# tangtang888/video-edge-ai-proxy

Measured on AMD Instinct MI355X. Metric: decoded FPS (whole node) + p50 VideoLatestImage latency, 256×1080p RTSP, higher is better.
Workload: dtype uint8 (BGR24 frames; bf16-capable consumer path)

## Files before the change

csrc/bindings.cpp:

```cpp
#include <malloc.h>

#include <pybind11/numpy.h>
#include <pybind11/pybind11.h>
#include <pybind11/stl.h>

#include "vep/hostprof.h"
#include "vep/avc.h"
#include "vep/avc_cavlc.h"
#include "vep/avc_recon.h"
#include "vep/bench_driver.h"
#include "vep/cabac.h"
#include "vep/codec.h"
#include "vep/gpu.h"
#include "vep/h264.h"
#include "vep/hevc_ctu.h"
#include "vep/hevc_dec.h"
#include "vep/hevc_kern.h"
#include "vep/jpeg.h"
#include "vep/scale.h"
#include "bind_ext.h"
#include "vep/runtime.h"
#include "vep/synth.h"

namespace py = pybind11;
// ... 113 lines not shown
  py::array_t<uint32_t> counts({py::ssize_t(r.rows), py::ssize_t(r.cols)});
  std::memcpy(counts.mutable_data(), r.counts.data(), r.counts.size() * sizeof(uint32_t));
  d["counts"] = counts;
  return d;
}

struct CpuDecoder {
  StreamParser parser;
  MbUpdate upd;
  HostSurface surf;
  PictureInfo last;
  avc::Decoder avc;
  std::vector<HostSurface> slots;
  bool general = false;
  int target = 0;
  int coded = 0;
  bool fields_out = false;
  HostSurface woven;
  mutable HostSurface weave_tmp;
  const HostSurface& out() const { return general ? (fields_out ? woven : slots[size_t(target)]) : surf; }
  const HostSurface& frame_of(const avc::OutFrame& f) const {
    if (!f.fields) return slots[size_t(f.slot)];
    avc::weave_fields(slots[2 * size_t(f.slot)], slots[2 * size_t(f.slot) + 1], weave_tmp);
    return weave_tmp;
  }
  py::object decode(const AccessUnit& au) {
    bool no_output = false;
    {
      py::gil_scoped_release nogil;
      bool done = false;
      if (!general) {
        try {
          upd.clear_payload();
          last = parser.parse(au, upd);
          if (surf.coded_w != last.coded_width || surf.coded_h != last.coded_height)
            surf.alloc(last.coded_width, last.coded_height);
          cpu_apply_update(upd, surf);
          coded = upd.nslots;
          done = true;
        } catch (const UnsupportedStream&) {
          if (au.codec != Codec::kH264) throw;
          general = true;
        }
      }
      std::vector<avc::OutFrame> outs;
      size_t nal = 0;
      while (!done) {
        avc::PicturePtr pic = avc.parse(au, 0, &nal);
        done = nal >= au.nals.size();
        if (slots.size() < size_t(pic->dpb_slots)) slots.resize(size_t(pic->dpb_slots));
        for (auto& h : slots)
          if (h.coded_w != pic->wmbs * 16 || h.coded_h != pic->hmbs * 16 || h.bd != pic->bd || h.cf != pic->cf)
            h.alloc(pic->wmbs * 16, pic->hmbs * 16, pic->bd, pic->cf);
        avc::cpu_reconstruct(*pic, slots);
        coded = pic->info.coded_mbs;
        pictures.push_back(pic->info);
        for (const avc::MbRec& m : pic->mbs) {
          ++kinds[m.kind];
          if (m.flags & avc::kMbT8x8) ++t8x8;
          if (m.flags & avc::kMbWp) ++weighted;
          if (m.kind <= avc::kInter) {
            bool bi = false, l1only = false;
            for (int k = 0; k < 4; ++k) {
              bi |= m.ref[k] != 0xFF && m.ref1[k] != 0xFF;
              l1only |= m.ref[k] == 0xFF && m.ref1[k] != 0xFF;
            }
            bipred += bi;
            list1_only += l1only;
          }
        }
        outs.insert(outs.end(), pic->outputs.begin(), pic->outputs.end());
        if (!done) continue;
        pending_outputs = outs;
        no_output = outs.empty();
        if (!no_output) {
          last = outs.back().info;
          target = outs.back().slot;
          fields_out = outs.back().fields;
          if (fields_out) woven = frame_of(outs.back());
          last_poc = outs.back().poc;
          last_pts = outs.back().au.pts;
        }
      }
    }
    if (no_output) return py::none();
    py::array_t<uint8_t> o({last.height, last.width, 3});
    cpu_nv12_to_bgr(out(), last.crop_left, last.crop_top, last.width, last.height, o.mutable_data());
    return o;
  }
  py::list frames_of(const std::vector<avc::OutFrame>& fs) const {
    py::list l;
    for (const auto& f : fs) {
      const HostSurface& s = frame_of(f);
      l.append(py::make_tuple(f.au.pts, surface_planes(s)));
    }
    return l;
  }
  py::list flush() {
    py::list out_list;
    for (const auto& f : avc.flush_output()) {
      py::array_t<uint8_t> o({f.info.height, f.info.width, 3});
      cpu_nv12_to_bgr(frame_of(f), f.info.crop_left, f.info.crop_top, f.info.width, f.info.height,
                      o.mutable_data());
      out_list.append(o);
    }
    return out_list;
// ... 668 lines not shown
        for (int i = 0; i < 16; ++i) want[256 + 16 * k + i] = res.blk[16 + k][i] = coded ? val(dens) : 0;
        if (coded) res.chroma |= u8(1u << k);
      }
      avc::Picture pic;
      pic.wmbs = pic.hmbs = 1;
      pic.mbs.resize(1);
      avc::MbRec rec{};
      rec.kind = res.t8 ? avc::kI8x8 : avc::kI16x16;
      rec.flags = res.t8 ? u8(avc::kMbT8x8) : u8(0);
      avc::MbState s;
      avc::store_mb(pic, 0, rec, s, &res, nullptr);
      i16 got[avc::kDenseCoefs];
      avc::expand_coefs(pic.coefs.data(), pic.mbs[0], got);
      bad_avc += std::memcmp(got, want, sizeof got) != 0 ||
                 pic.coefs.size() != size_t(avc::coef_words(pic.mbs[0])) + avc::coef_values(pic.coefs.data(), pic.mbs[0]);
      for (int log2 = 2; log2 <= 5; ++log2) {
        const int nn = 1 << (2 * log2);
        std::vector<i16> dense(size_t(nn), 0), val_list, out(size_t(nn + nn / 16)), back(static_cast<size_t>(nn));
        std::vector<u16> pos;
        for (int k = 0; k < nn; ++k)
          if ((dense[size_t(k)] = val(dens))) pos.push_back(u16(k));
        for (size_t i = pos.size(); i > 1; --i) std::swap(pos[i - 1], pos[size_t(rnd() % i)]);
        for (u16 k : pos) val_list.push_back(dense[k]);
        const int n = hevc::hk_sparse_store(log2, pos.data(), val_list.data(), int(pos.size()), out.data());
        hevc::hk_sparse_expand(out.data(), log2, back.data());
        bad_hevc += back != dense || n != hevc::hk_sparse_words(log2) + int(pos.size());
      }
    }
    return std::make_pair(bad_avc, bad_hevc);
  });
  m.def("avc_parse_seconds", [](const std::vector<std::shared_ptr<AccessUnit>>& aus, int reps) {
    py::gil_scoped_release r;
    double best = 1e30;
    for (int k = 0; k < std::max(1, reps); ++k) {
      avc::Decoder dec;
      const i64 t0 = mono_us();
      for (const auto& au : aus) {
        size_t nal = 0;
        do dec.parse(*au, 0, &nal);
        while (nal < au->nals.size());
      }
      best = std::min(best, double(mono_us() - t0) * 1e-6);
    }
    return best;
  }, py::arg("aus"), py::arg("reps") = 3);
  m.def("avc_record_stats", [](const std::vector<std::shared_ptr<AccessUnit>>& aus) {
    py::gil_scoped_release r;
    avc::Decoder dec;
    u64 mbs = 0, coefs = 0, nz = 0, mvs = 0, pics = 0;
    for (const auto& au : aus) {
      auto p = dec.parse(*au);
      if (!p) continue;
      ++pics;
      mbs += p->mbs.size();
      coefs += p->coefs.size();
      mvs += p->mvs.size();
      for (const avc::MbRec& m : p->mbs)
        if (m.kind != avc::kIPcm) nz += avc::coef_values(p->coefs.data(), m);
    }
    py::gil_scoped_acquire g;
    py::dict d;
    d["pictures"] = pics;
    d["mbs"] = mbs;
    d["coefs"] = coefs;
    d["nonzero"] = nz;
    d["mvs"] = mvs;
    return d;
  });
  m.def("hevc_record_stats", [](const std::vector<std::shared_ptr<AccessUnit>>& aus) {
    py::gil_scoped_release r;
    hevc::Decoder dec;
    dec.set_gpu_mode(true);
    u64 pics = 0, tus = 0, coefs = 0, nz = 0, pus = 0;
    for (const auto& au : aus) {
      dec.decode(*au);
      for (const auto& p : dec.take_gpu_pictures()) {
        ++pics;
        tus += p->tus.size();
        pus += p->pus.size();
        coefs += p->coefs.size();
        for (i16 c : p->coefs) nz += c != 0;
      }
    }
    py::gil_scoped_acquire g;
    py::dict d;
    d["pictures"] = pics;
    d["tus"] = tus;
    d["coefs"] = coefs;
    d["nonzero"] = nz;
    d["pus"] = pus;
    return d;
  });
  m.def("avc_intra8x8_tap_check", [](u64 seed, int trials) {
    u64 st = seed * 0x9E3779B97F4A7C15ull + 7;
    auto rnd = [&]() {
      st ^= st << 13;
      st ^= st >> 7;
      st ^= st << 17;
      return int(st & 255);
    };
    int bad = 0;
    for (int t = 0; t < trials; ++t) {
      int s[25];
      for (int k = 0; k < 25; ++k) s[k] = (t & 3) == 0 ? (rnd() & 1) * 255 : rnd();
      auto T = [&](int i) { return s[1 + i]; };
      auto L = [&](int j) { return j < 0 ? s[0] : s[17 + j]; };
// ... 1064 lines not shown
          return tiles;
        },
        py::arg("pics"), py::arg("stream"));
  m.def("letterbox",
        [](uintptr_t y, uintptr_t uv, int pitch, int src_w, int src_h, int crop_left, int crop_top,
           int size, uintptr_t out_hwc, uintptr_t out_chw, int chw_dtype, std::vector<float> mean,
           std::vector<float> stdv, int pad, uintptr_t stream, int format) {
          gpu::LetterboxDesc d{};
          d.y = reinterpret_cast<const u8*>(y);
          d.uv = reinterpret_cast<const u8*>(uv);
          d.pitch = pitch;
          d.src_w = src_w;
          d.src_h = src_h;
          d.crop_left = crop_left;
          d.crop_top = crop_top;
          d.out_hwc = reinterpret_cast<u8*>(out_hwc);
          d.out_chw = reinterpret_cast<void*>(out_chw);
          gpu::LetterboxParams p{};
          p.format = format;
          p.size = size;
          p.chw_dtype = chw_dtype;
          for (int k = 0; k < 3; ++k) {
            p.mean[k] = mean.size() == 3 ? mean[size_t(k)] : 0.f;
            p.inv_std[k] = 1.f / (stdv.size() == 3 ? stdv[size_t(k)] : 1.f);
          }
          p.pad_value = u8(pad);
          gpu::check_letterbox(d, p);
          gpu::fill_letterbox_geometry(d, size, format == gpu::kLbNV12);
          gpu::launch_letterbox_one(d, p, reinterpret_cast<hipStream_t>(stream));
        },
        py::arg("y"), py::arg("uv"), py::arg("pitch"), py::arg("src_w"), py::arg("src_h"),
        py::arg("crop_left"), py::arg("crop_top"), py::arg("size"), py::arg("out_hwc"),
        py::arg("out_chw"), py::arg("chw_dtype"), py::arg("mean"), py::arg("std"), py::arg("pad"),
        py::arg("stream"), py::arg("format") = 0);
  m.def("nv12_to_chw",
        [](uintptr_t in, uintptr_t out, int n, int size, int chw_dtype, std::vector<float> mean,
           std::vector<float> stdv, uintptr_t stream) {
          float m3[3], is3[3];
          for (int k = 0; k < 3; ++k) {
            m3[k] = mean.size() == 3 ? mean[size_t(k)] : 0.f;
            is3[k] = 1.f / (stdv.size() == 3 ? stdv[size_t(k)] : 1.f);
          }
          gpu::launch_nv12_to_chw(reinterpret_cast<const u8*>(in), reinterpret_cast<void*>(out), n,
                                  size, chw_dtype, m3, is3, reinterpret_cast<hipStream_t>(stream));
        });
  m.def("letterbox_geometry", [](int src_w, int src_h, int size, bool even) {
    gpu::LetterboxDesc d{};
    d.src_w = src_w;
    d.src_h = src_h;
    gpu::fill_letterbox_geometry(d, size, even);
    return py::make_tuple(d.nw, d.nh, d.pad_x, d.pad_y);
  }, py::arg("src_w"), py::arg("src_h"), py::arg("size"), py::arg("even") = false);

  bind_net(m);
  bind_mux(m);
  bind_hevc(m);
  bind_bus(m);
  bind_rpc(m);
}
```

csrc/vep/avc.cpp:

```cpp
#include "avc.h"

#include <immintrin.h>

#include <algorithm>
#include <array>

#include "avc_cavlc.h"
#include "avc_internal.h"
#include "fanout.h"

namespace vep::avc {

using h264::Pps;
using h264::Sps;


void MbNeighbours::reset(int wmbs, int hmbs, bool ring) {
  w_ = wmbs;
  h_ = hmbs;
  cur_ = -1;
  run_slice_ = ~0u;
  run_start_ = 0;
  announced_ = 0;
  const size_t n = size_t(wmbs) * hmbs;
  if (++epoch_ == 0) {
    epoch_ = 1;
    stamp_.clear();
  }
  size_t ns = n;
  mask_ = ~size_t(0);
  if (ring) {
    size_t r = 1;
    while (r < 2 * (size_t(wmbs) + 2)) r <<= 1;
    if (r < n) {
      ns = r;
      mask_ = r - 1;
    }
  }
  if (st_.size() != ns) st_.assign(ns, MbState{});
  if (tag_.size() != ns) tag_.assign(ns, ~0u);
  if (stamp_.size() != n) stamp_.assign(n, 0u);
}

static int coded_count(const MbState& s, int blk) {
  if (s.kind == kSkip) return 0;
  if (s.kind == kIPcm) return 16;
  return s.tc[blk];
}

int MbNeighbours::nc_luma(int mb, int blk) const {
  const int bx = blk & 3, by = blk >> 2;
  int na = -1, nb = -1;
  const int am = mb_at(mb, bx * 4 - 1, by * 4);
  if (am >= 0) na = coded_count(st_[size_t(am) & mask_], bx > 0 ? blk - 1 : blk + 3);
  const int bm = mb_at(mb, bx * 4, by * 4 - 1);
  if (bm >= 0) nb = coded_count(st_[size_t(bm) & mask_], by > 0 ? blk - 4 : blk + 12);
  if (na >= 0 && nb >= 0) return (na + nb + 1) >> 1;
  if (na >= 0) return na;
// ... 1184 lines not shown
  Picture& pic_;
  const SliceCtx& sc_;
  const u8* pcm_ = nullptr;
};

}

namespace {

bool legacy_slice(const SliceHdr& sh, const Sps& sps, const Pps& pps) {
  return !pps.cabac && !sh.field_pic && sps.chroma_format_idc == 1 && sps.bit_depth_luma == 8 && (sh.type() == h264::kP || sh.type() == h264::kI) && !pps.transform_8x8_mode &&
         !sps.scaling_matrix_present && !pps.scaling_matrix_present && !sh.explicit_wp &&
         pps.chroma_qp_index_offset == pps.second_chroma_qp_index_offset;
}

int dpb_slots_for(const Sps& sps) {
  int bound;
  if (sps.max_num_reorder_frames >= 0) bound = sps.max_num_reorder_frames;
  else if (sps.poc_type == 2 || sps.profile_idc == 66) bound = 0;
  else bound = sps.max_dpb_frames();
  return std::min(kMaxDpbSlots, std::max(1, sps.max_num_ref_frames) + bound + 2);
}

}

static void validate_picture(const Picture& p);

struct Decoder::SliceUnit {
  MbNeighbours nb;
  Picture shard;
  ColBuild colb;
  std::vector<u8> rbsp;
  SliceHdr sh;
  const Sps* sps = nullptr;
  const Pps* pps = nullptr;
  size_t bitpos = 0;
  int slice_idx = 0;
  std::vector<ListEntry> list[2];
  std::array<std::vector<u32>, 2> uids;
};

PicturePtr Decoder::parse(const AccessUnit& au, i64 tag, size_t* next_nal) {
  struct FenceOnExit {
    ~FenceOnExit() {
#if defined(__x86_64__)
      _mm_sfence();
#endif
    }
  } fence;
  auto pic = pic_pool_->acquire([](Picture& p) {
    auto mbs = std::move(p.mbs);
    auto coefs = std::move(p.coefs), mvs = std::move(p.mvs);
    auto wps = std::move(p.wps);
    std::vector<OutFrame> outputs = std::move(p.outputs);
    p = Picture{};
    coefs.clear();
    mvs.clear();
    wps.clear();
    outputs.clear();
    p.mbs = std::move(mbs);
    p.coefs = std::move(coefs);
    p.mvs = std::move(mvs);
    p.wps = std::move(wps);
    p.outputs = std::move(outputs);
  });
  bool got = false;
  bool hard_flush = false;
  bool second_field = false;
  int slice_idx = 0;
  SliceHdr first;
  const Sps* act_sps = nullptr;
  const Pps* act_pps = nullptr;
  std::vector<u8> scratch;
  std::vector<std::array<std::vector<u32>, 2>> slice_uids;
  ColBuild colb;
  std::shared_ptr<ColMotion> col_built;
  struct ColbGuard {
    Picture* p;
    ~ColbGuard() { p->colb = nullptr; }
  } colb_guard{pic.get()};
  int nslices = 0;
  for (size_t i = 0; i < au.nals.size(); ++i)
    if (au.nal_size(i) >= 2) {
      const int t = h264::nal_type(au.nal(i)[0]);
      nslices += (t == h264::kNalSlice || t == h264::kNalIdr) ? 1 : 0;
    }
  const bool par = parallel_slices_ && nslices >= 2 && FanOut::shared().size() > 0;
  int nunits = 0;
  const size_t start = next_nal ? *next_nal : 0;
  if (next_nal) *next_nal = au.nals.size();
  for (size_t i = start; i < au.nals.size(); ++i) {
    const u8* p = au.nal(i);
    const size_t n = au.nal_size(i);
    if (n < 2) continue;
    const int t = h264::nal_type(p[0]);
    if (t == h264::kNalSps || t == h264::kNalPps) {
      size_t rn;
      const u8* r = unescape(p, n, epb_, scratch, rn);
      if (t == h264::kNalSps) {
        Sps s = h264::parse_sps(r, rn);
        check_sps_supported(s);
        sps_[s.sps_id] = s;
      } else {
        Pps q = h264::parse_pps(r, rn);
        pps_[q.pps_id] = q;
      }
      continue;
    }
// ... 107 lines not shown
          pair_.f.fields = true;
        }
        pair_.have |= u8(1 << int(sh.bottom_field));
        pair_.poc[int(sh.bottom_field)] = pic->poc;
      } else {
        pic->target = pick_slot();
      }
      if (sh.nal_ref_idc != 0 && sps.profile_idc != 66) {
        col_built = col_pool_->acquire([](ColMotion&) {});
        col_built->wmbs = W;
        col_built->hmbs = Hp;
        col_built->corners = sps.direct_8x8;
        col_built->b.resize(size_t(W) * Hp * size_t(sps.direct_8x8 ? 4 : 16));
        colb.col = col_built.get();
        pic->colb = &colb;
      }
      got = true;
    } else {
      VEP_CHECK(&sps == act_sps, "slices of one picture reference different SPSs");
      if (sh.field_pic != first.field_pic || sh.bottom_field != first.bottom_field) {
        VEP_CHECK(next_nal != nullptr, "H.264: one access unit holds several pictures");
        *next_nal = i;
        break;
      }
      if (sh.type() == h264::kB || pic->info.pict_type == 'I') pic->info.pict_type = "PBISi"[sh.type()];
    }
    if (sh.field_pic) build_field_lists(sh, sps, pic->poc);
    else build_lists(sh, sps, pic->poc);
    std::array<std::vector<u32>, 2> uids;
    for (int l = 0; l < 2; ++l)
      for (const auto& e : list_[l]) uids[size_t(l)].push_back(e.uid);
    slice_uids.push_back(std::move(uids));
    colb.set_uids(&slice_uids.back());
    if (par) {
      if (units_.size() <= size_t(nunits)) units_.push_back(std::make_unique<SliceUnit>());
      SliceUnit& u = *units_[size_t(nunits++)];
      u.rbsp.assign(r + 1, r + rn);
      u.sh = sh;
      u.sps = &sps;
      u.pps = &pps;
      u.bitpos = br.pos();
      u.slice_idx = slice_idx;
      u.list[0] = list_[0];
      u.list[1] = list_[1];
      u.uids = slice_uids.back();
    } else {
      parse_slice_data(nb_, *pic, sh, sps, pps, r + 1, rn - 1, br.pos(), slice_idx, list_);
    }
    ++slice_idx;
    VEP_CHECK(slice_idx < 65535, "too many slices");
  }
  VEP_CHECK(got, "access unit has no slice");
  (void)act_pps;
  std::vector<u8> covered;
  if (par) {
    const int W = pic->wmbs, H = pic->hmbs;
    ColMotion* col_target = colb.col;
    FanOut::shared().run(nunits, [&](int k) {
      SliceUnit& u = *units_[size_t(k)];
      u.nb.reset(W, H, true);
      Picture& sh = u.shard;
      sh.wmbs = W;
      sh.hmbs = H;
      if (sh.mbs.size() != size_t(W) * H) sh.mbs.assign(size_t(W) * H, MbRec{});
      sh.coefs.clear();
      sh.mvs.clear();
      sh.wps.clear();
      sh.intra_mbs = sh.intra_res = sh.inter_mbs = 0;
      sh.deblock = false;
      sh.target = pic->target;
      sh.dpb_slots = pic->dpb_slots;
      sh.constrained_intra = pic->constrained_intra;
      sh.poc = pic->poc;
      sh.bd = pic->bd;
      sh.cf = pic->cf;
      sh.qp_bias = pic->qp_bias;
      sh.qpc_bias = pic->qpc_bias;
      u.colb.col = col_target;
      u.colb.set_uids(&u.uids);
      sh.colb = col_target ? &u.colb : nullptr;
      parse_slice_data(u.nb, sh, u.sh, *u.sps, *u.pps, u.rbsp.data(), u.rbsp.size(), u.bitpos, u.slice_idx, u.list);
#if defined(__x86_64__)
      _mm_sfence();
#endif
    });
    parallel_slices_run_ += u64(nunits);
    covered.assign(size_t(pic->nmbs()), 0);
    for (int k = 0; k < nunits; ++k) {
      SliceUnit& u = *units_[size_t(k)];
      const Picture& sh = u.shard;
      const u32 coef0 = u32(pic->coefs.size()), mv0 = u32(pic->mvs.size()), wp0 = u32(pic->wps.size());
      const u32 res0 = u32(pic->intra_res);
      pic->coefs.insert(pic->coefs.end(), sh.coefs.begin(), sh.coefs.end());
      pic->mvs.insert(pic->mvs.end(), sh.mvs.begin(), sh.mvs.end());
      pic->wps.insert(pic->wps.end(), sh.wps.begin(), sh.wps.end());
      pic->intra_mbs += sh.intra_mbs;
      pic->intra_res += sh.intra_res;
      pic->inter_mbs += sh.inter_mbs;
      pic->deblock |= sh.deblock;
      for (int mb = u.sh.first_mb; mb < pic->nmbs(); ++mb) {
        if (!u.nb.announced(mb)) continue;
        VEP_CHECK(!covered[size_t(mb)], "H.264: slices overlap");
        covered[size_t(mb)] = 1;
        MbRec m = sh.mbs[size_t(mb)];
        m.coef += coef0;
        if (m.kind == kSkip || m.kind == kInter) m.mv += mv0;
        if (m.flags & kMbWp) m.wp += wp0;
        if (m.res != kNoRes) m.res += res0;
        pic->mbs[size_t(mb)] = m;
      }
    }
  }
  int ncovered = 0;
  if (par)
    for (u8 c : covered) ncovered += c;
  auto announced = [&](int mb) { return par ? covered[size_t(mb)] != 0 : nb_.announced(mb); };
  int missing = 0;
  for (int mb = 0; (par ? ncovered : nb_.announced_count()) < pic->nmbs() && mb < pic->nmbs(); ++mb) {
    MbRec& m = pic->mbs[size_t(mb)];
    if (announced(mb)) continue;
    ++missing;
    if (pic->colb) colb.none(mb);
    m = MbRec{};
    m.res = kNoRes;
    m.dbk = 1;
    m.slice = u16(0xFFFF);
    std::fill(std::begin(m.ref1), std::end(m.ref1), u8(0xFF));
    if (!dpb_.empty()) {
      m.kind = kSkip;
      int cs = dpb_.front().slot;
      if (pic->structure) {
        const int par = pic->structure - 1;
        cs = 2 * cs + ((((dpb_.front().fields | dpb_.front().lt_fields) >> par) & 1) ? par : 1 - par);
      }
      for (auto& rf : m.ref) rf = u8(cs);
      m.mv = u32(pic->mvs.size());
      m.flags |= kMbMv16;
      pic->mvs.resize(pic->mvs.size() + 2, 0);
      ++pic->inter_mbs;
    } else {
      m.kind = kI16x16;
      m.i16_mode = 2;
      std::fill(std::begin(m.ref), std::end(m.ref), u8(0xFF));
      ++pic->intra_mbs;
    }
  }
  pic->info.coded_mbs = pic->nmbs() - missing;
  const u32 uid = next_uid_++;
  if (first.field_pic) {
    if (first.nal_ref_idc != 0)
      mark_field(first, *act_sps, pic->target >> 1, pic->poc, uid, second_field && pair_.ref, std::move(col_built));
    if (first.has_mmco5() && !second_field) {
      pic->poc = 0;
      pair_.frame_num = 0;
      pair_.poc[int(first.bottom_field)] = 0;
      pair_.boundary = true;
      pair_.hard = reorder_cur_ == 0;
    }
    if (second_field) close_pair(*pic);
  } else {
    if (first.nal_ref_idc != 0) {
      mark_references(first, *act_sps, pic->target, pic->poc, uid, std::move(col_built));
    }
    const bool boundary = first.idr() || first.has_mmco5();
    if (first.has_mmco5()) pic->poc = 0;
    bump(*pic, out_of(*pic), boundary, boundary && (hard_flush || reorder_cur_ == 0));
  }
  if (missing || par) validate(*pic);
  else validate_picture(*pic);
  return pic;
}

Decoder::Decoder() {
  if (const char* e = std::getenv("VEP_AVC_SLICE_THREADS")) parallel_slices_ = e[0] != '0';
}
Decoder::~Decoder() = default;

void Decoder::parse_slice_data(MbNeighbours& nb, Picture& pic, const SliceHdr& sh, const Sps& sps, const Pps& pps,
                               const u8* data, size_t n, size_t bitpos, int slice_idx,
                               const std::vector<ListEntry> (&lists)[2]) {
  if (legacy_slice(sh, sps, pps)) {
    Bits br(data, n, bitpos);
    const size_t stop = BitReader(data, n).stop_bit_pos();
    SliceCtx sc{sh, pps, slice_idx, sh.type() == h264::kP, sh.qp, lists[0]};
    const int total = pic.nmbs();
    int mb = sh.first_mb;
    VEP_CHECK(mb < total, "first_mb_in_slice past end of picture");
    bool more = true;
    while (more) {
      if (sc.is_p) {
        const u32 run = br.ue();
        VEP_CHECK(u32(total - mb) >= run, "mb_skip_run past end of picture");
        MbDecoder d(nb, pic, sc);
        for (u32 k = 0; k < run; ++k) d.skip(mb++);
        if (run > 0) {
          more = br.pos() < stop;
          if (!more) break;
        }
      }
      VEP_CHECK(mb < total, "macroblock address past end of picture");
      MbDecoder d(nb, pic, sc);
      d.macroblock(br, mb);
      if (d.qp_out_ >= 0) sc.qp = d.qp_out_;
      VEP_CHECK(!br.overrun(), "slice data overrun");
      more = br.pos() < stop;
      ++mb;
    }
    return;
  }
  SliceEnv env;
  env.sh = &sh;
  env.sps = &sps;
  env.pps = &pps;
  env.slice = slice_idx;
  env.list[0] = &lists[0];
  env.list[1] = &lists[1];
  env.cur_poc = pic.poc;
  env.scaling = h264::resolve_scaling(sps, pps);
  env.field = sh.field_pic;
  decode_slice_generic(nb, pic, env, data, n, bitpos);
}

static inline void validate_mb(const Picture& p, const MbRec& m, bool written = false) {
  const size_t ncoef = p.coefs.size(), nmv = p.mvs.size();
  VEP_CHECK(m.kind <= kI8x8, "macroblock kind out of range");
  VEP_CHECK(p.cf == 2 || m.chroma_coded < 0x100, "chroma block mask out of range");
  VEP_CHECK(m.qp <= 51 + p.qp_bias && m.qpc <= 51 + p.qpc_bias && m.qpc2 <= 51 + p.qpc_bias,
            "macroblock QP out of range");
  if (m.kind == kIPcm) {
    const size_t ns = p.cf == 2 ? size_t(kPcmMaxSamples) : size_t(kPcmMbBytes);
    VEP_CHECK(size_t(m.coef) + (p.bd > 8 ? ns : ns / 2) <= ncoef, "I_PCM samples outside the pool");
    return;
  }
  const size_t nw = size_t(coef_words(m));
  VEP_CHECK(size_t(m.coef) + nw <= ncoef, "coefficient masks outside the pool");
  VEP_CHECK(written || size_t(m.coef) + nw + coef_values(p.coefs.data(), m) <= ncoef, "coefficients outside the pool");
  VEP_CHECK(m.chroma_mode <= 3 && m.i16_mode <= 3, "intra prediction mode out of range");
  if (m.flags & kMbT8x8)
    for (int q = 0; q < 4; ++q) {
      const u32 g = (u32(m.luma_coded) >> ((q & 1) * 2 + (q >> 1) * 8)) & 0x33u;
      VEP_CHECK(g == 0 || g == 0x33u, "8x8 residual block partially coded");
    }
  if (m.kind == kSkip || m.kind == kInter) {
    VEP_CHECK(size_t(m.mv) + size_t(mv_per_list(m.flags)) * ((m.flags & kMbL1) ? 2 : 1) <= nmv,
              "motion vectors outside the pool");
    for (int k = 0; k < 4; ++k) {
      const int r0 = m.ref[k], r1 = m.ref1[k];
      VEP_CHECK(r0 != 0xFF || r1 != 0xFF, "inter partition without a reference");
      VEP_CHECK((r0 == 0xFF || r0 < p.dpb_slots) && (r1 == 0xFF || r1 < p.dpb_slots),
                "reference slot outside the DPB");
      VEP_CHECK(r1 == 0xFF || (m.flags & kMbL1), "list-1 reference without list-1 motion");
    }
    if (m.flags & kMbWp) VEP_CHECK(size_t(m.wp) + 4 <= p.wps.size(), "weights outside the pool");
  } else if (m.kind == kI4x4) {
    for (u8 b : m.i4) VEP_CHECK((b & 15) <= 8 && (b >> 4) <= 8, "Intra_4x4 mode out of range");
  } else if (m.kind == kI8x8) {
    VEP_CHECK((m.flags & kMbT8x8) && (m.i4[0] & 15) <= 8 && (m.i4[0] >> 4) <= 8 && (m.i4[1] & 15) <= 8 &&
                  (m.i4[1] >> 4) <= 8,
              "Intra_8x8 mode out of range");
  }
  VEP_CHECK(m.res == kNoRes || (is_intra(m.kind) && m.res < u32(p.intra_res)), "residual slot out of range");
}

static inline void validate_written_mb(const Picture& p, const MbRec& m) {
  const size_t ncoef = p.coefs.size(), nmv = p.mvs.size();
  bool ok = (m.kind <= kI8x8) & (p.cf == 2 || m.chroma_coded < 0x100) & (m.qp <= 51 + p.qp_bias) &
            (m.qpc <= 51 + p.qpc_bias) & (m.qpc2 <= 51 + p.qpc_bias);
  if (m.kind != kIPcm) {
    ok &= size_t(m.coef) + size_t(coef_words(m)) <= ncoef;
    ok &= (m.chroma_mode <= 3) & (m.i16_mode <= 3);
    if (m.flags & kMbT8x8)
      for (int q = 0; q < 4; ++q) {
        const u32 g = (u32(m.luma_coded) >> ((q & 1) * 2 + (q >> 1) * 8)) & 0x33u;
        ok &= (g == 0) | (g == 0x33u);
      }
    if (m.kind == kSkip || m.kind == kInter) {
      ok &= size_t(m.mv) + size_t(mv_per_list(m.flags)) * ((m.flags & kMbL1) ? 2 : 1) <= nmv;
      u32 r0w, r1w;
      std::memcpy(&r0w, m.ref, 4);
      std::memcpy(&r1w, m.ref1, 4);
      for (int k = 0; k < 4; ++k) {
        const u32 r0 = (r0w >> (8 * k)) & 0xFFu, r1 = (r1w >> (8 * k)) & 0xFFu;
        ok &= (r0 != 0xFF) | (r1 != 0xFF);
        ok &= (r0 == 0xFF) | (r0 < u32(p.dpb_slots));
        ok &= (r1 == 0xFF) | (r1 < u32(p.dpb_slots));
        ok &= (r1 == 0xFF) | ((m.flags & kMbL1) != 0);
      }
      if (m.flags & kMbWp) ok &= size_t(m.wp) + 4 <= p.wps.size();
    } else if (m.kind == kI4x4 || m.kind == kI8x8) {
      for (u8 b : m.i4) ok &= ((b & 15) <= 8) & ((b >> 4) <= 8);
      if (m.kind == kI8x8) ok &= (m.flags & kMbT8x8) != 0;
    }
    ok &= m.res == kNoRes || (is_intra(m.kind) && m.res < u32(p.intra_res));
  }
  if (!ok) validate_mb(p, m, true);
}

static void validate_picture(const Picture& p) {
  VEP_CHECK(p.dpb_slots >= 1 && p.dpb_slots <= kMaxDpbSlots && p.target >= 0 && p.target < p.dpb_slots,
            "picture DPB slots out of range");
  VEP_CHECK(p.wmbs > 0 && p.hmbs > 0 && p.mbs.size() == size_t(p.nmbs()), "picture size mismatch");
}

void validate(const Picture& p) {
  validate_picture(p);
  for (const MbRec& m : p.mbs) validate_mb(p, m);
}


static inline void stream_words(void* dst, const void* src, size_t bytes) {
#if defined(__x86_64__)
  long long w[16];
  for (size_t o = 0; o < bytes; o += sizeof w) {
    const size_t n = bytes - o < sizeof w ? bytes - o : sizeof w;
    std::memcpy(w, static_cast<const char*>(src) + o, n);
    long long* d = reinterpret_cast<long long*>(static_cast<char*>(dst) + o);
    for (size_t k = 0; k < n / 8; ++k) _mm_stream_si64(d + k, w[k]);
  }
#else
  std::memcpy(dst, src, bytes);
#endif
}

void ColBuild::none(int mb) {
  const int per = col->corners ? 4 : 16;
  ColMotion::Blk* out = &col->b[size_t(mb) * size_t(per)];
  for (int k = 0; k < per; ++k) out[k] = ColMotion::Blk{{0, 0}, 0u, i8(-1)};
}

void ColBuild::store(int mb, const MbState& st) {
  if (is_intra(st.kind) || !uids) {
    none(mb);
    return;
  }
  static constexpr u8 kCorner[4] = {0, 3, 12, 15};
  const auto& lu = *uids;
  if (col->corners) {
    ColMotion::Blk out[4];
    for (int k = 0; k < 4; ++k) {
      const int l = st.ref[0][k] >= 0 ? 0 : 1;
      const int ri = st.ref[l][k];
      out[k] = ri < 0 ? ColMotion::Blk{{0, 0}, 0u, i8(-1)}
                      : ColMotion::Blk{{st.mv[l][kCorner[k]][0], st.mv[l][kCorner[k]][1]}, uid_tab[l][ri & 31], i8(ri)};
    }
    stream_words(&col->b[size_t(mb) * 4], out, sizeof out);
    return;
  }
  ColMotion::Blk* out = &col->b[size_t(mb) * 16];
  for (int blk = 0; blk < 16; ++blk) {
    const int b8 = ((blk >> 3) << 1) | ((blk & 3) >> 1);
    const int l = st.ref[0][b8] >= 0 ? 0 : 1;
    const int ri = st.ref[l][b8];
    if (ri < 0) {
      out[blk] = ColMotion::Blk{{0, 0}, 0u, i8(-1)};
      continue;
    }
    out[blk] = ColMotion::Blk{{st.mv[l][blk][0], st.mv[l][blk][1]},
                              size_t(ri) < lu[size_t(l)].size() ? lu[size_t(l)][size_t(ri)] : 0u, i8(ri)};
  }
}

std::shared_ptr<ColMotion> build_col_motion(const MbNeighbours& nb, int wmbs, int hmbs,
                                            const std::vector<std::array<std::vector<u32>, 2>>& slice_uids,
                                            bool corners, Recycler<ColMotion>* pool) {
  auto col = pool ? pool->acquire([](ColMotion&) {}) : std::make_shared<ColMotion>();
  col->wmbs = wmbs;
  col->hmbs = hmbs;
  col->corners = corners;
  const int per = corners ? 4 : 16;
  col->b.resize(size_t(wmbs) * hmbs * size_t(per));
  static constexpr u8 kCorner[4] = {0, 3, 12, 15};
  for (int mb = 0; mb < wmbs * hmbs; ++mb) {
    const MbState& st = nb.at(mb);
    ColMotion::Blk* out = &col->b[size_t(mb) * size_t(per)];
    if (!nb.decoded(mb) || is_intra(st.kind) || slice_uids.empty()) {
      for (int k = 0; k < per; ++k) out[k] = ColMotion::Blk{{0, 0}, 0u, i8(-1)};
      continue;
    }
    const auto& lu = slice_uids[std::min<size_t>(st.slice, slice_uids.size() - 1)];
    for (int k = 0; k < per; ++k) {
      const int blk = corners ? kCorner[k] : k;
      const int b8 = ((blk >> 3) << 1) | ((blk & 3) >> 1);
      const int l = st.ref[0][b8] >= 0 ? 0 : 1;
      const int ri = st.ref[l][b8];
      if (ri < 0) {
        out[k] = ColMotion::Blk{{0, 0}, 0u, i8(-1)};
        continue;
      }
      out[k] = ColMotion::Blk{{st.mv[l][blk][0], st.mv[l][blk][1]},
                              size_t(ri) < lu[size_t(l)].size() ? lu[size_t(l)][size_t(ri)] : 0u, i8(ri)};
    }
  }
  return col;
}

namespace {
template <class P>
// ... 153 lines not shown
      int k = 0;
      for (int i = 0; i < 8; ++i)
        if ((m >> i) & 1) {
          c[m][2 * k] = u8(2 * i);
          c[m][2 * k + 1] = u8(2 * i + 1);
          ++k;
        }
      for (int j = 2 * k; j < 16; ++j) c[m][j] = 0x80;
    }
  }
};
static constexpr Compact8 kCompact8{};

static inline i16* compact16(const i16* p, u32 mask, i16* out) {
#if defined(__SSSE3__)
  const __m128i lo = _mm_loadu_si128(reinterpret_cast<const __m128i*>(p));
  const __m128i hi = _mm_loadu_si128(reinterpret_cast<const __m128i*>(p + 8));
  const u32 m0 = mask & 0xFFu, m1 = mask >> 8;
  _mm_storeu_si128(reinterpret_cast<__m128i*>(out),
                   _mm_shuffle_epi8(lo, _mm_load_si128(reinterpret_cast<const __m128i*>(kCompact8.c[m0]))));
  out += __builtin_popcount(m0);
  _mm_storeu_si128(reinterpret_cast<__m128i*>(out),
                   _mm_shuffle_epi8(hi, _mm_load_si128(reinterpret_cast<const __m128i*>(kCompact8.c[m1]))));
  return out + __builtin_popcount(m1);
#else
  for (int i = 0; i < 16; ++i) {
    *out = p[i];
    out += (mask >> i) & 1;
  }
  return out;
#endif
}

static inline u32 motion_uniformity(const i16* mv) {
#if defined(__AVX2__)
  const __m256i a = _mm256_loadu_si256(reinterpret_cast<const __m256i*>(mv));
  const __m256i b = _mm256_loadu_si256(reinterpret_cast<const __m256i*>(mv + 16));
  const __m256i v0 = _mm256_broadcastd_epi32(_mm256_castsi256_si128(a));
  const __m256i tl = _mm256_setr_epi32(0, 0, 2, 2, 0, 0, 2, 2);
  const u32 all = u32(_mm256_movemask_epi8(_mm256_and_si256(_mm256_cmpeq_epi32(a, v0), _mm256_cmpeq_epi32(b, v0))));
  const u32 q8 = u32(_mm256_movemask_epi8(_mm256_and_si256(_mm256_cmpeq_epi32(a, _mm256_permutevar8x32_epi32(a, tl)),
                                                           _mm256_cmpeq_epi32(b, _mm256_permutevar8x32_epi32(b, tl)))));
  return (all == 0xFFFFFFFFu ? 1u : 0u) | (q8 == 0xFFFFFFFFu ? 2u : 0u);
#else
  u32 v[16];
  std::memcpy(v, mv, sizeof v);
  bool u16 = true, u8x8 = true;
  for (int b = 1; b < 16; ++b) u16 &= v[b] == v[0];
  for (int b = 0; b < 16; ++b) u8x8 &= v[b] == v[((b >> 3) << 3) | (b & 2)];
  return (u16 ? 1u : 0u) | (u8x8 ? 2u : 0u);
#endif
}

static inline void store_motion(Picture& pic, MbRec& m, const MbState& s) {
  const int nl = (m.flags & kMbL1) ? 2 : 1;
  u32 u = 3;
  for (int l = 0; l < nl; ++l) u &= motion_uniformity(&s.mv[l][0][0]);
  m.flags |= (u & 1) ? kMbMv16 : ((u & 2) ? kMbMv8x8 : 0);
  m.mv = u32(pic.mvs.size());
  const int per = (u & 1) ? 2 : ((u & 2) ? 8 : 32);
  i16* out = pic.mvs.extend(size_t(per * nl));
  for (int l = 0; l < nl; ++l, out += per) {
    const i16* v = &s.mv[l][0][0];
    if (per == 2) {
      std::memcpy(out, v, 4);
    } else if (per == 8) {
      std::memcpy(out, v, 4);
      std::memcpy(out + 2, v + 4, 4);
      std::memcpy(out + 4, v + 16, 4);
      std::memcpy(out + 6, v + 20, 4);
    } else {
      std::memcpy(out, v, 64);
    }
  }
}

static inline void store_rec(MbRec* dst, const MbRec& m) {
  static_assert(sizeof(MbRec) % 8 == 0 && sizeof(ColMotion::Blk) * 4 % 8 == 0, "8-byte words");
  stream_words(dst, &m, sizeof(MbRec));
}

void store_skip_mb(Picture& pic, int mb, MbRec& m, const MbState& s) {
  m.coef = u32(pic.coefs.size());
  m.luma_coded = 0;
  m.chroma_coded = 0;
  m.wp = 0;
  m.res = kNoRes;
  store_motion(pic, m, s);
  ++pic.inter_mbs;
  if (!(m.dbk & 1)) pic.deblock = true;
  for (int k = 0; k < 4; ++k) {
    const int r0 = m.ref[k], r1 = m.ref1[k];
    VEP_CHECK((r0 != 0xFF || r1 != 0xFF) && (r0 == 0xFF || r0 < pic.dpb_slots) && (r1 == 0xFF || r1 < pic.dpb_slots) &&
                  (r1 == 0xFF || (m.flags & kMbL1)),
              "skipped macroblock reference slot outside the DPB");
  }
  VEP_CHECK(m.qp <= 51 + pic.qp_bias && m.qpc <= 51 + pic.qpc_bias && m.qpc2 <= 51 + pic.qpc_bias,
            "macroblock QP out of range");
  store_rec(&pic.mbs[size_t(mb)], m);
  if (pic.colb) pic.colb->store(mb, s);
}

void store_mb(Picture& pic, int mb, MbRec m, const MbState& s, const MbResidual* res, const u8* pcm,
              const WpEntry* wp) {
  m.coef = u32(pic.coefs.size());
  m.luma_coded = 0;
  m.chroma_coded = 0;
  if (m.kind == kIPcm) {
    VEP_CHECK(pcm, "I_PCM macroblock without samples");
    const size_t ns = pic.cf == 2 ? size_t(kPcmMaxSamples) : size_t(kPcmMbBytes);
    const size_t o = pic.coefs.size(), nb = pic.bd > 8 ? 2 * ns : ns;
    pic.coefs.resize(o + nb / 2);
    std::memcpy(pic.coefs.data() + o, pcm, nb);
  } else if (res && (res->luma | res->chroma)) {
    m.luma_coded = res->luma;
    m.chroma_coded = res->chroma;
    if (res->t8) m.flags |= kMbT8x8;
    const i16* grp[32];
    int ng = 0;
    if (res->t8) {
      for (int q = 0; q < 4; ++q)
        if ((res->luma >> ((q & 1) * 2 + (q >> 1) * 8)) & 1)
          for (int w = 0; w < 4; ++w) grp[ng++] = res->b8[q] + 16 * w;
    } else {
      for (u32 w = res->luma; w; w &= w - 1) grp[ng++] = res->blk[__builtin_ctz(w)];
    }
    for (u32 w = res->chroma; w; w &= w - 1) grp[ng++] = res->blk[16 + __builtin_ctz(w)];
    u16 mask[32];
    int nv = 0;
    for (int g = 0; g < ng; ++g) {
      mask[g] = nonzero_mask16(grp[g]);
      nv += __builtin_popcount(mask[g]);
    }
    const size_t o = pic.coefs.size();
    i16* out = pic.coefs.extend(size_t(ng + nv) + 8);
    std::memcpy(out, mask, size_t(ng) * sizeof(u16));
    i16* v = out + ng;
    for (int g = 0; g < ng; ++g) v = compact16(grp[g], mask[g], v);
    pic.coefs.resize(o + size_t(ng + nv));
  }
  m.mv = 0;
  m.wp = 0;
  m.flags &= u8(~(kMbMv8x8 | kMbMv16));
  if (m.kind == kSkip || m.kind == kInter) {
    store_motion(pic, m, s);
    if (wp && (m.flags & kMbWp)) {
      m.wp = u32(pic.wps.size());
      pic.wps.insert(pic.wps.end(), wp, wp + 4);
    } else {
      m.flags &= u8(~kMbWp);
    }
    ++pic.inter_mbs;
  } else if (m.kind == kIPcm) {
    ++pic.inter_mbs;
  } else {
    ++pic.intra_mbs;
  }
  m.res = is_intra(m.kind) && m.kind != kIPcm && (m.luma_coded | m.chroma_coded) ? u32(pic.intra_res++) : kNoRes;
  if (!(m.dbk & 1)) pic.deblock = true;
  validate_written_mb(pic, m);
  store_rec(&pic.mbs[size_t(mb)], m);
  if (pic.colb) pic.colb->store(mb, s);
}


namespace {

bool intra_avail(const Picture& pic, const MbRec& m, int nx, int ny) {
  if (nx < 0 || ny < 0 || nx >= pic.wmbs) return false;
  const MbRec& n = pic.mbs[size_t(ny) * pic.wmbs + nx];
  if (n.slice != m.slice) return false;
  return !(pic.constrained_intra && !is_intra(n.kind));
}

const i16* luma_res(const i16* dense, const MbRec& m, int r) {
  if (!((m.luma_coded >> r) & 1)) return nullptr;
  return dense + 16 * r;
}

const i16* chroma_res(const i16* dense, const MbRec& m, int c, int b, int nbc) {
  const int k = c * nbc + b;
  if (!((m.chroma_coded >> k) & 1)) return nullptr;
  return dense + 256 + 16 * k;
}

void luma_residual(const i16* dense, const MbRec& m, int* out) {
  std::memset(out, 0, 256 * sizeof(int));
  if (m.flags & kMbT8x8) {
    for (int q = 0; q < 4; ++q) {
      if (!((m.luma_coded >> ((q & 1) * 2 + (q >> 1) * 8)) & 1)) continue;
      int r[64];
      idct8x8(dense + 64 * q, r);
      for (int i = 0; i < 8; ++i)
        for (int j = 0; j < 8; ++j) out[((q >> 1) * 8 + i) * 16 + (q & 1) * 8 + j] = r[i * 8 + j];
    }
    return;
  }
  for (int blk = 0; blk < 16; ++blk) {
// ... 235 lines not shown
  const bool cf2 = T.cf == 2;
  P* Yp = yplane<P>(T);
  P* UV = uvplane<P>(T);
  auto mvs = [&](const MbRec& r) { return is_intra(r.kind) ? kZeroMv : &pic.mvs[size_t(r.mv)]; };
  for (int mb = 0; mb < pic.nmbs(); ++mb) {
    const MbRec& q = pic.mbs[size_t(mb)];
    if (q.dbk & 1) continue;
    const int mx = mb % W, my = mb / W;
    const bool left = mx > 0 && !((q.dbk & 2) && pic.mbs[size_t(mb - 1)].slice != q.slice);
    const bool top = my > 0 && !((q.dbk & 2) && pic.mbs[size_t(mb - W)].slice != q.slice);
    const i16* mq = mvs(q);
    for (int dir = 0; dir < 2; ++dir) {
      for (int e = 0; e < 4; ++e) {
        if (e == 0 && !(dir == 0 ? left : top)) continue;
        const MbRec& p = e > 0 ? q : pic.mbs[size_t(dir == 0 ? mb - 1 : mb - W)];
        const i16* mp = mvs(p);
        const bool luma_edge = !((e & 1) && (q.flags & kMbT8x8));
        const bool chroma_edge = cf2 ? (dir == 1 || !(e & 1)) : !(e & 1);
        if (!luma_edge && !chroma_edge) continue;
        const EdgeParams ep = edge_params(p.qp - qb, q.qp - qb, q.alpha_off, q.beta_off, bd);
        const EdgeParams epcs[2] = {edge_params(p.qpc - qcb, q.qpc - qcb, q.alpha_off, q.beta_off, bd),
                                    edge_params(p.qpc2 - qcb, q.qpc2 - qcb, q.alpha_off, q.beta_off, bd)};
        int bs[16];
        for (int k = 0; k < 16; ++k) {
          const int bq = dir == 0 ? (k >> 2) * 4 + e : e * 4 + (k >> 2);
          const int bp = e > 0 ? (dir == 0 ? bq - 1 : bq - 4) : (dir == 0 ? bq + 3 : bq + 12);
          bs[k] = boundary_strength(p, bp, mp, q, bq, mq, e == 0, pic.structure != 0, dir == 0);
        }
        for (int k = 0; k < 16 && luma_edge; ++k) {
          if (!bs[k]) continue;
          if (dir == 0) filter_line(Yp + size_t(my * 16 + k) * pitch + mx * 16 + 4 * e, 1, bs[k], ep, false, bd);
          else filter_line(Yp + size_t(my * 16 + 4 * e) * pitch + mx * 16 + k, long(pitch), bs[k], ep, false, bd);
        }
        if (!chroma_edge) continue;
        const int ch = cf2 ? 16 : 8;
        for (int c = 0; c < 2; ++c)
          for (int k = 0; k < (dir == 0 ? ch : 8); ++k) {
            const EdgeParams& epc = epcs[c];
            const int b = bs[dir == 0 && cf2 ? k : 2 * k];
            if (!b) continue;
            if (dir == 0)
              filter_line(UV + size_t(my * ch + k) * pitch + (mx * 8 + 2 * e) * 2 + c, 2, b, epc, true, bd);
            else
              filter_line(UV + size_t(my * ch + (cf2 ? 4 : 2) * e) * pitch + (mx * 8 + k) * 2 + c, long(pitch), b,
                          epc, true, bd);
          }
      }
    }
  }
}
}

void cpu_reconstruct_mb(const Picture& pic, int mb, std::vector<HostSurface>& slots) {
  if (slots[size_t(pic.target)].wide()) reconstruct_mb_t<u16>(pic, mb, slots);
  else reconstruct_mb_t<u8>(pic, mb, slots);
}

void cpu_deblock(const Picture& pic, HostSurface& T) {
  if (T.wide()) deblock_t<u16>(pic, T);
  else deblock_t<u8>(pic, T);
}

void weave_fields(const HostSurface& top, const HostSurface& bottom, HostSurface& frame) {
  VEP_CHECK(top.coded_w == bottom.coded_w && top.coded_h == bottom.coded_h && !top.wide(), "weave: field sizes");
  const int w = top.coded_w, fh = top.coded_h;
  if (frame.coded_w != w || frame.coded_h != 2 * fh) frame.alloc(w, 2 * fh);
  for (int r = 0; r < 2 * fh; ++r)
    std::memcpy(&frame.y[size_t(r) * w], &(r & 1 ? bottom : top).y[size_t(r >> 1) * w], size_t(w));
  for (int r = 0; r < fh; ++r)
    std::memcpy(&frame.uv[size_t(r) * w], &(r & 1 ? bottom : top).uv[size_t(r >> 1) * w], size_t(w));
}

void cpu_reconstruct(const Picture& pic, std::vector<HostSurface>& slots) {
  VEP_CHECK(pic.target >= 0 && pic.target < int(slots.size()), "target slot out of range");
  HostSurface& T = slots[size_t(pic.target)];
  VEP_CHECK(T.coded_w == pic.wmbs * 16 && T.coded_h == pic.hmbs * 16 && T.bd == pic.bd && T.cf == pic.cf,
            "surface size mismatch");
  for (int mb = 0; mb < pic.nmbs(); ++mb) cpu_reconstruct_mb(pic, mb, slots);
  if (pic.deblock) cpu_deblock(pic, T);
}

}
```

csrc/vep/avc.h:

```cpp
#pragma once

#include <array>
#include <map>
#include <memory>

#include "hostmem.h"
#include "recycle.h"
#include "avc_recon.h"
#include "codec.h"

namespace vep::avc {

constexpr int kMaxDpbSlots = 34;

struct AuMeta {
  i64 pts = 0, dts = 0, arrival_ms = 0;
  i64 tag = 0;
  bool keyframe = false, corrupt = false;
};

struct OutFrame {
  int slot = -1;
  PictureInfo info;
  AuMeta au;
  int poc = 0;
  bool fields = false;
};

struct ColBuild;

struct Picture {
  int wmbs = 0, hmbs = 0;
  hostmem::pinned_vector<MbRec> mbs;
  hostmem::pinned_vector<i16> coefs;
  hostmem::pinned_vector<i16> mvs;
  hostmem::pinned_vector<WpEntry> wps;
  int target = 0;
  int dpb_slots = 1;
  int structure = 0;
  int bd = 8, qp_bias = 0, qpc_bias = 0;
  int cf = 1;
  bool second_field = false;
  bool constrained_intra = false;
  int intra_mbs = 0;
  int intra_res = 0;
  int inter_mbs = 0;
  bool deblock = false;
  bool idr = false;
  int poc = 0;
  PictureInfo info;
  AuMeta au;
  std::vector<OutFrame> outputs;
  ColBuild* colb = nullptr;

  int nmbs() const { return wmbs * hmbs; }
};
using PicturePtr = std::shared_ptr<const Picture>;

void validate(const Picture& p);

struct SliceHdr {
  int nal_type = 0, nal_ref_idc = 0;
  int first_mb = 0, slice_type = 0, pps_id = 0, frame_num = 0, idr_pic_id = 0;
  bool field_pic = false, bottom_field = false;
  int redundant_pic_cnt = 0;
  int poc_lsb = 0, delta_poc_bottom = 0, delta_poc[2] = {0, 0};
  bool direct_spatial = true;
  int num_ref_idx[2] = {1, 1};
  struct RefMod {
    int idc, val;
  };
  std::vector<RefMod> ref_mods[2];
  bool explicit_wp = false;
  int luma_lwd = 0, chroma_lwd = 0;
  struct Weight {
    i16 w[3], o[3];
  };
  std::vector<Weight> wt[2];
  bool no_output_of_prior_pics = false, long_term_reference = false;
  bool adaptive_marking = false;
  struct Mmco {
    int op, a, b;
  };
  std::vector<Mmco> mmcos;
  int cabac_init_idc = 0;
  int qp = 26;
  int disable_deblocking = 0, alpha_off = 0, beta_off = 0;
  bool idr() const { return nal_type == h264::kNalIdr; }
  int type() const { return slice_type % 5; }
  bool has_mmco5() const {
    for (const auto& m : mmcos)
      if (m.op == 5) return true;
    return false;
  }
};

struct MbState {
  u8 kind = 0xFF;
  u8 skip = 0;
  u8 direct16 = 0;
  u8 direct8 = 0;
  u8 t8x8 = 0;
  u8 cbp = 0;
  u8 chroma_mode = 0;
  u8 qp = 0;
  u16 slice = 0;
  u16 cbf = 0;
  u8 cbf_dc = 0;
  u8 cbf_cac[2] = {0, 0};
  i8 ref[2][4] = {{-1, -1, -1, -1}, {-1, -1, -1, -1}};
  i16 mv[2][16][2] = {};
  u8 mvd[2][16][2] = {};
  u8 tc[16] = {};
  u8 tcc[2][8] = {};
  u8 i4[16] = {};
};

class MbNeighbours {
 public:
  void reset(int wmbs, int hmbs, bool ring = false);
  void begin(int mb);
  MbState& at(int mb) { return st_[size_t(mb) & mask_]; }
  const MbState& at(int mb) const { return st_[size_t(mb) & mask_]; }
  int wmbs() const { return w_; }
  int hmbs() const { return h_; }
  int mb_at(int mb, int x, int y) const;
  bool mb_available(int mb, int nb) const {
    const size_t i = size_t(nb) & mask_;
    return nb >= 0 && stamp_[size_t(nb)] == epoch_ && tag_[i] == u32(nb) && st_[i].kind != 0xFF &&
           st_[i].slice == st_[size_t(mb) & mask_].slice;
  }
  bool decoded(int mb) const {
    return stamp_[size_t(mb)] == epoch_ && tag_[size_t(mb) & mask_] == u32(mb) && st_[size_t(mb) & mask_].kind != 0xFF;
  }
  bool announced(int mb) const { return stamp_[size_t(mb)] == epoch_; }
  int announced_count() const { return announced_; }
  int nc_luma(int mb, int blk) const;
  int nc_chroma(int mb, int c, int blk, int nbc = 4) const;
  int pred_intra4x4(int mb, int blk, bool constrained_intra) const;
  int pred_intra8x8(int mb, int b8, bool constrained_intra) const;
  void pred_mv(int mb, int x4, int y4, int w4, int h4, int list, int ref, u16 done, int shape,
               int out[2]) const;
  void pred_mv(int mb, int x4, int y4, int w4, int h4, int ref, u16 done, int shape, int out[2]) const {
    pred_mv(mb, x4, y4, w4, h4, 0, ref, done, shape, out);
  }
  void pskip_mv(int mb, int out[2]) const;
  void mb_neighbour_refs(int mb, int list, int ref[3]) const;
  void direct_spatial_pred(int mb, int list, int& ref, int mv[2]) const;
  void direct_spatial_both(int ref[2], int mv[2][2]) const;

 private:
  struct Nb {
    bool avail;
    int ref;
    int mv[2];
  };
  Nb motion_at(int mb, int x, int y, u16 done, int list) const;
  void nb16(int list, Nb n[3]) const;
  void pred_mv16(int list, int ref, int out[2]) const;
  int w_ = 0, h_ = 0;
  int cur_ = -1, cx_ = 0, cy_ = 0, a_ = -1, b_ = -1, c_ = -1, d_ = -1;
  u32 run_slice_ = ~0u;
  int run_start_ = 0;
  u32 epoch_ = 0;
  int announced_ = 0;
  size_t mask_ = ~size_t(0);
  std::vector<u32> stamp_;
  std::vector<u32> tag_;
  std::vector<MbState> st_;
};

inline void MbNeighbours::begin(int mb) {
  int mx, my;
  const int prev = cur_;
  const bool next = mb == prev + 1 && prev >= 0;
  if (mb == prev) {
    mx = cx_;
    my = cy_;
  } else if (next) {
    mx = cx_ + 1;
    my = cy_;
    if (mx == w_) {
      mx = 0;
      ++my;
    }
  } else {
    mx = mb % w_;
    my = mb / w_;
  }
  cur_ = mb;
  cx_ = mx;
  cy_ = my;
  if (stamp_[size_t(mb)] != epoch_) {
    stamp_[size_t(mb)] = epoch_;
    ++announced_;
  }
  tag_[size_t(mb) & mask_] = u32(mb);
  const u32 sl = st_[size_t(mb) & mask_].slice;
  if (next && sl == run_slice_) {
    const int f = run_start_;
    a_ = mx > 0 && mb - 1 >= f ? mb - 1 : -1;
    b_ = my > 0 && mb - w_ >= f ? mb - w_ : -1;
// ... 83 lines not shown
  }
}

inline void MbNeighbours::direct_spatial_both(int ref[2], int mv[2][2]) const {
  const int nm[3] = {a_, b_, c_ >= 0 ? c_ : d_};
  const int nblk[3] = {3, 12, c_ >= 0 ? 12 : 15};
  bool avail[3];
  int r[2][3];
  int v[2][3][2];
  for (int k = 0; k < 3; ++k) {
    avail[k] = nm[k] >= 0;
    for (int l = 0; l < 2; ++l) {
      r[l][k] = -1;
      v[l][k][0] = v[l][k][1] = 0;
    }
    if (!avail[k]) continue;
    const MbState& s = st_[size_t(nm[k]) & mask_];
    if (is_intra(s.kind)) continue;
    const int b8 = ((nblk[k] >> 3) << 1) | ((nblk[k] & 3) >> 1);
    for (int l = 0; l < 2; ++l) {
      r[l][k] = s.ref[l][b8];
      if (r[l][k] < 0) continue;
      v[l][k][0] = s.mv[l][nblk[k]][0];
      v[l][k][1] = s.mv[l][nblk[k]][1];
    }
  }
  auto minpos = [](int a, int b) { return (a >= 0 && b >= 0) ? (a < b ? a : b) : (a > b ? a : b); };
  const bool only_a = !avail[1] && !avail[2] && avail[0];
  for (int l = 0; l < 2; ++l) {
    const int rf = minpos(r[l][0], minpos(r[l][1], r[l][2]));
    ref[l] = rf;
    mv[l][0] = mv[l][1] = 0;
    if (rf < 0) continue;
    if (only_a) {
      mv[l][0] = v[l][0][0];
      mv[l][1] = v[l][0][1];
      continue;
    }
    const int match = (r[l][0] == rf) + (r[l][1] == rf) + (r[l][2] == rf);
    if (match == 1) {
      const int k = r[l][0] == rf ? 0 : (r[l][1] == rf ? 1 : 2);
      mv[l][0] = v[l][k][0];
      mv[l][1] = v[l][k][1];
      continue;
    }
    for (int c = 0; c < 2; ++c) {
      const int a = v[l][0][c], b = v[l][1][c], d = v[l][2][c];
      const int lo = a < b ? a : b, hi = a < b ? b : a;
      mv[l][c] = d < lo ? lo : (d > hi ? hi : d);
    }
  }
}

struct ColMotion {
  struct Blk {
    i16 mv[2];
    u32 pid;
    i8 ref;
  };
  int wmbs = 0, hmbs = 0;
  bool corners = false;
  std::vector<Blk> b;
  size_t index(int mb, int blk) const {
    return corners ? size_t(mb) * 4 + size_t(((blk >> 3) << 1) | ((blk & 3) >> 1)) : size_t(mb) * 16 + size_t(blk);
  }
};

struct ColBuild {
  ColMotion* col = nullptr;
  const std::array<std::vector<u32>, 2>* uids = nullptr;
  u32 uid_tab[2][32] = {};
  void set_uids(const std::array<std::vector<u32>, 2>* u) {
    uids = u;
    for (int l = 0; l < 2; ++l)
      for (size_t k = 0; k < 32; ++k) uid_tab[l][k] = u && k < (*u)[size_t(l)].size() ? (*u)[size_t(l)][k] : 0u;
  }
  void store(int mb, const MbState& st);
  void none(int mb);
};

struct RefPic {
  int slot = -1;
  int frame_num = 0;
  int frame_num_wrap = 0;
  bool long_term = false;
  int lt_idx = 0;
  int poc = 0;
  u32 uid = 0;
  std::shared_ptr<const ColMotion> col;
  u8 fields = 3;
  u8 lt_fields = 0;
  int poc_f[2] = {0, 0};
  u32 uid_f[2] = {0, 0};
  std::shared_ptr<const ColMotion> col_f[2];
};

struct ListEntry {
  int slot = -1;
  int poc = 0;
  bool long_term = false;
  u32 uid = 0;
  const ColMotion* col = nullptr;
};

class Decoder {
 public:
  PicturePtr parse(const AccessUnit& au, i64 tag = 0, size_t* next_nal = nullptr);
  void absorb_parameter_sets(const AccessUnit& au);
  bool has_sps() const { return !sps_.empty(); }
  void reset_references();
  int dpb_slots() const { return dpb_slots_; }
  int pending_output() const { return int(pending_.size()); }
  std::vector<OutFrame> flush_output();

 private:
  struct Pending {
    OutFrame f;
    u32 epoch;
  };
  void build_lists(const SliceHdr& sh, const h264::Sps& sps, int cur_poc);
  void build_field_lists(const SliceHdr& sh, const h264::Sps& sps, int cur_poc);
  void mark_field(const SliceHdr& sh, const h264::Sps& sps, int slot, int poc, u32 uid, bool second,
                  std::shared_ptr<const ColMotion> col);
  void mark_references(const SliceHdr& sh, const h264::Sps& sps, int slot, int poc, u32 uid,
                       std::shared_ptr<const ColMotion> col);
  int pick_slot() const;
  int compute_poc(const SliceHdr& sh, const h264::Sps& sps);
  void bump(Picture& pic, const OutFrame& f, bool new_epoch, bool hard);
  OutFrame out_of(const Picture& pic) const;
  int reorder_depth(const h264::Sps& sps) const;
  void parse_slice_data(MbNeighbours& nb, Picture& pic, const SliceHdr& sh, const h264::Sps& sps,
                        const h264::Pps& pps, const u8* data, size_t n, size_t bitpos, int slice_idx,
                        const std::vector<ListEntry> (&lists)[2]);

  std::map<int, h264::Sps> sps_;
  std::map<int, h264::Pps> pps_;
  std::vector<u8> rbsp_;
  std::vector<u32> epb_;
  MbNeighbours nb_;
  std::vector<RefPic> dpb_;
  std::shared_ptr<Recycler<Picture>> pic_pool_ = Recycler<Picture>::make(12);
  std::shared_ptr<Recycler<ColMotion>> col_pool_ = Recycler<ColMotion>::make(8);
  std::vector<Pending> pending_;
  std::vector<ListEntry> list_[2];
  int max_lt_idx_ = -1;
  int dpb_slots_ = 2;
  int wmbs_ = 0, hmbs_ = 0;
  int bd_ = 8;
  int cf_ = 1;
  bool have_idr_ = false;
  int pinned_slot_ = -1;
  int last_out_poc_ = 0;
  i64 last_out_epoch_ = -1;
  u32 epoch_ = 0;
  int adaptive_reorder_ = 0;
  int reorder_cur_ = 0;
  u32 next_uid_ = 1;
  int prev_poc_msb_ = 0, prev_poc_lsb_ = 0;
  int prev_frame_num_ = 0, prev_frame_num_offset_ = 0;
  bool prev_ref_mmco5_ = false;
  std::vector<std::vector<MbState>> spare_;
  struct SliceUnit;
  bool parallel_slices_ = true;
  std::vector<std::unique_ptr<SliceUnit>> units_;
  u64 parallel_slices_run_ = 0;
  bool field_mode_ = false;
  struct OpenPair {
    bool open = false;
    int slot = -1, frame_num = 0, bottom = 0;
    int poc[2] = {0, 0};
    bool ref = false, boundary = false, hard = false;
    u8 have = 0;
    OutFrame f;
  } pair_;
  void close_pair(Picture& pic);

 public:
  Decoder();
  ~Decoder();
  u64 parallel_slices_run() const { return parallel_slices_run_; }
  u64 mmco_ops[7] = {0, 0, 0, 0, 0, 0, 0};
  u64 list_mods = 0, long_term_marked = 0;
  u64 redundant_slices_skipped = 0;
};

void cpu_reconstruct(const Picture& pic, std::vector<HostSurface>& slots);
void weave_fields(const HostSurface& top, const HostSurface& bottom, HostSurface& frame);

struct MbLevels {
  int luma[16][16];
  int dc[16];
  int cdc[2][4];
  int cac[2][4][16];
  u16 lmask = 0;
  u8 cmask = 0;
  u8 dcmask = 0;
  void update_masks() {
    lmask = cmask = dcmask = 0;
    for (int r = 0; r < 16; ++r)
      for (int k = 0; k < 16; ++k)
        if (luma[r][k]) lmask |= u16(1u << r);
    for (int k = 0; k < 16; ++k)
      if (dc[k]) dcmask |= 1;
    for (int c = 0; c < 2; ++c)
      for (int b = 0; b < 4; ++b) {
        if (cdc[c][b]) dcmask |= u8(2 << c);
        for (int k = 0; k < 16; ++k)
          if (cac[c][b][k]) cmask |= u8(1u << (c * 4 + b));
      }
  }
};
struct MbResidual {
  i16 blk[32][16];
  i16 b8[4][64];
  u16 luma = 0;
  u16 chroma = 0;
  bool t8 = false;
};
void dequantize_mb(const MbLevels& lv, bool i16x16, int qp, int qpc, MbResidual& out);
void store_mb(Picture& pic, int mb, MbRec m, const MbState& s, const MbResidual* res, const u8* pcm,
              const WpEntry* wp = nullptr);
void store_skip_mb(Picture& pic, int mb, MbRec& m, const MbState& s);
void cpu_reconstruct_mb(const Picture& pic, int mb, std::vector<HostSurface>& slots);
void cpu_deblock(const Picture& pic, HostSurface& target);
void intra4x4_neighbours(const Picture& pic, int mb, int idx, const HostSurface& T, Intra4Nb& n);
void intra16_neighbours(const Picture& pic, int mb, const HostSurface& T, Intra16Nb& n);
void chroma_neighbours(const Picture& pic, int mb, int c, const HostSurface& T, IntraChromaNb& n);
void intra8x8_neighbours(const Picture& pic, int mb, int q, const HostSurface& T, int* f, bool& has_top,
                         bool& has_left);

class StreamEncoder {
 public:
  virtual ~StreamEncoder() = default;
// ... 97 lines not shown
```

csrc/vep/avc_mb.cpp:

```cpp
#include <algorithm>
#include <memory>
#include <cstddef>
#include <cstring>

#include "avc_cabac.h"
#include "avc_cavlc.h"
#include "avc_internal.h"

namespace vep::avc {

namespace {

struct Dequant {
  int ls4[6][6][16];
  int ls8[2][6][64];
  explicit Dequant(const h264::ScalingLists& sl) {
    for (int l = 0; l < 6; ++l)
      for (int m = 0; m < 6; ++m)
        for (int k = 0; k < 16; ++k) {
          const int pos = kZigzag4x4[k];
          ls4[l][m][pos] = int(sl.l4[l][k]) * norm_adjust(m, pos >> 2, pos & 3);
        }
    for (int l = 0; l < 2; ++l)
      for (int m = 0; m < 6; ++m)
// ... 56 lines not shown
          if ((*lst)[k].slot >= 0) slot_[l][k + 1] = u8((*lst)[k].slot);
    }
    for (int q = 0; q < 52 + qpbd_ && q < int(std::size(qpc_tab_[0])); ++q) {
      qpc_tab_[0][q] = u8(chroma_qp_bd(q - qpbd_, pps_.chroma_qp_index_offset, qpbdc_) + qpbdc_);
      qpc_tab_[1][q] = u8(chroma_qp_bd(q - qpbd_, pps_.second_chroma_qp_index_offset, qpbdc_) + qpbdc_);
    }
    fast_direct_ = !kWrite && type_ == h264::kB && sh_.direct_spatial && sps_.direct_8x8 && !weighted_;
  }

  Bits* br = nullptr;
  BitWriter* bw = nullptr;
  Bins* bins = nullptr;
  cabac::Decoder* cabac = nullptr;
  cabac::Encoder* cenc = nullptr;
  const MbDesc* want = nullptr;
  int prev_qpd_nz = 0;

  int qp() const { return qp_; }

  int ue(u32 v) {
    if constexpr (kWrite) {
      bw->ue(v);
      return int(v);
    } else {
      return int(br->ue());
    }
  }
  int se(int v) {
    if constexpr (kWrite) {
      bw->se(v);
      return v;
    } else {
      return br->se();
    }
  }
  int u(int n, u32 v) {
    if constexpr (kWrite) {
      bw->u(n, v);
      return int(v);
    } else {
      return int(br->u(n));
    }
  }

  static void clear_but_mv(MbState& s) {
    static const MbState z{};
    std::memcpy(static_cast<void*>(&s), &z, offsetof(MbState, mv));
    std::memcpy(static_cast<void*>(&s.mvd), &z.mvd, sizeof(MbState) - offsetof(MbState, mvd));
  }

  bool read_skip_flag(int mb, bool v = false) {
    MbState& s = nb_.at(mb);
    if constexpr (kWrite) s = MbState{};
    else clear_but_mv(s);
    s.slice = u16(env_.slice);
    nb_.begin(mb);
    auto cond = [&](int m) { return m >= 0 && !nb_.at(m).skip ? 1 : 0; };
    const int inc = cond(nb_.mb_at(mb, -1, 0)) + cond(nb_.mb_at(mb, 0, -1));
    return bins->mb_skip(type_ == h264::kB, inc, v) != 0;
  }

  void skip_mb(int mb, bool fresh) {
    MbState& s = nb_.at(mb);
    if (fresh) {
      s = MbState{};
      s.slice = u16(env_.slice);
      nb_.begin(mb);
    }
    s.kind = kSkip;
    s.skip = 1;
    s.qp = u8(qp_ + qpbd_);
    MbResidual res;
    res.luma = 0;
    res.chroma = 0;
    if (type_ == h264::kP) {
      s.ref[0][0] = s.ref[0][1] = s.ref[0][2] = s.ref[0][3] = 0;
      need_ref(0, 0);
      int mv[2];
      nb_.pskip_mv(mb, mv);
      for (auto& v : s.mv[0]) {
        v[0] = i16(mv[0]);
        v[1] = i16(mv[1]);
      }
    } else {
      s.direct16 = 1;
      s.direct8 = 0xF;
      if (fast_direct_) direct16_spatial(mb, s);
      else direct(mb, s, 0xF);
    }
    prev_qpd_nz = 0;
    if (!weighted_ && !kWrite) emit_skip(mb, s);
    else emit(mb, s, res, 0, 0, nullptr);
  }

  void coded_mb(int mb, bool fresh) {
    MbState& s = nb_.at(mb);
    if (fresh) {
      s = MbState{};
      s.slice = u16(env_.slice);
      nb_.begin(mb);
    } else if constexpr (!kWrite) {
      std::memset(static_cast<void*>(s.mv), 0, sizeof s.mv);
    }
    int mbt = read_mb_type(mb, kWrite ? want->mb_type : 0);
    int itype = -1;
    if (type_ == h264::kI) {
      itype = mbt;
    } else if (type_ == h264::kP) {
      VEP_CHECK(mbt <= 30, "bad P mb_type");
      if (mbt >= 5) itype = mbt - 5;
    } else {
      VEP_CHECK(mbt <= 48, "bad B mb_type");
      if (mbt >= 23) itype = mbt - 23;
    }
    VEP_CHECK(itype <= 25, "bad intra mb_type");
    MbResidual res;
    res.luma = 0;
    res.chroma = 0;
    if (itype == 25) {
      pcm_mb(mb, s, res);
      return;
    }
    int cbp = 0, i16_mode = 0;
    const bool intra = itype >= 0;
    bool no_small = true;
    if (itype == 0) {
      if (pps_.transform_8x8_mode) s.t8x8 = u8(read_t8x8(mb, kWrite && want->t8x8));
      s.kind = s.t8x8 ? kI8x8 : kI4x4;
      intra_modes(mb, s);
      s.chroma_mode = u8(read_chroma_mode(mb, kWrite ? want->chroma_mode : 0));
    } else if (itype > 0) {
      s.kind = kI16x16;
      i16_mode = (itype - 1) % 4;
      cbp = (((itype - 1) / 4) % 3) << 4 | (itype >= 13 ? 15 : 0);
      std::fill(std::begin(s.i4), std::end(s.i4), u8(2));
      s.chroma_mode = u8(read_chroma_mode(mb, kWrite ? want->chroma_mode : 0));
      VEP_CHECK(!mono() || (cbp >> 4) == 0, "4:0:0: Intra_16x16 type with chroma coefficients");
    } else {
      s.kind = kInter;
      no_small = inter_pred(mb, s, mbt);
    }
    VEP_CHECK(s.chroma_mode <= 3, "bad intra_chroma_pred_mode");
    if (s.kind != kI16x16) cbp = read_cbp(mb, s, intra, kWrite ? want->cbp : 0);
    s.cbp = u8(cbp);
    if (s.kind == kInter && (cbp & 15) && pps_.transform_8x8_mode && no_small &&
        !(type_ == h264::kB && mbt == 0 && !sps_.direct_8x8))
      s.t8x8 = u8(read_t8x8(mb, kWrite && want->t8x8));
    int qp = qp_;
    if ((cbp & 15) || (cbp >> 4) || s.kind == kI16x16) {
      const int dqp = read_qp_delta(kWrite ? want->qp_delta : 0);
      VEP_CHECK(dqp >= -(26 + qpbd_ / 2) && dqp <= 25 + qpbd_ / 2, "mb_qp_delta out of range");
      qp = (qp + dqp + 52 + 2 * qpbd_) % (52 + qpbd_) - qpbd_;
      prev_qpd_nz = dqp != 0;
    } else {
      prev_qpd_nz = 0;
// ... 521 lines not shown
        if (cb.ref >= 0) {
          mvc[0] = cb.mv[0];
          mvc[1] = cb.mv[1];
          r0 = -1;
          for (size_t k = 0; k < l0.size() && r0 < 0; ++k)
            if (l0[k].slot >= 0 && l0[k].uid == cb.pid) r0 = int(k);
          if (r0 < 0) r0 = 0;
        }
        need_ref(0, r0);
        const ListEntry& p0 = l0[size_t(r0)];
        int m0[2], m1[2];
        const int td = clip3i(-128, 127, c1.poc - p0.poc);
        if (td == 0 || p0.long_term) {
          m0[0] = mvc[0];
          m0[1] = mvc[1];
          m1[0] = m1[1] = 0;
        } else {
          const int tb = clip3i(-128, 127, env_.cur_poc - p0.poc);
          const int tx = (16384 + std::abs(td / 2)) / td;
          const int dsf = clip3i(-1024, 1023, (tb * tx + 32) >> 6);
          for (int k = 0; k < 2; ++k) {
            m0[k] = (dsf * mvc[k] + 128) >> 8;
            m1[k] = m0[k] - mvc[k];
          }
        }
        fill(0, b8, blk, clip3i(-32768, 32767, m0[0]), clip3i(-32768, 32767, m0[1]));
        fill(1, b8, blk, clip3i(-32768, 32767, m1[0]), clip3i(-32768, 32767, m1[1]));
      }
      s.ref[0][b8] = i8(r0);
      s.ref[1][b8] = 0;
    }
  }

  void direct16_spatial(int mb, MbState& s) {
    if (!dcol_) {
      VEP_CHECK(env_.list[1] && !env_.list[1]->empty() && (*env_.list[1])[0].slot >= 0,
                "direct prediction without a list-1 reference");
      const ListEntry& c1 = (*env_.list[1])[0];
      VEP_CHECK(c1.col && c1.col->wmbs == nb_.wmbs() && c1.col->hmbs == nb_.hmbs() && c1.col->corners,
                "colocated picture motion missing");
      dcol_ = c1.col;
      dcol_long_ = c1.long_term;
    }
    int ref[2], mvp[2][2];
    nb_.direct_spatial_both(ref, mvp);
    const bool zero = ref[0] < 0 && ref[1] < 0;
    if (zero) ref[0] = ref[1] = 0;
    u32 pv[2];
    for (int l = 0; l < 2; ++l) {
      if (ref[l] >= 0) need_ref(l, ref[l]);
      const bool use = ref[l] >= 0 && !zero;
      pv[l] = use ? (u32(u16(mvp[l][0])) | u32(u16(mvp[l][1])) << 16) : 0u;
      std::memset(s.ref[l], ref[l], 4);
    }
    const ColMotion::Blk* cb = &dcol_->b[size_t(mb) * 4];
    u32 v8[2][4];
    for (int b8 = 0; b8 < 4; ++b8) {
      const bool col_zero = !dcol_long_ && cb[b8].ref == 0 && cb[b8].mv[0] >= -1 && cb[b8].mv[0] <= 1 &&
                            cb[b8].mv[1] >= -1 && cb[b8].mv[1] <= 1;
      for (int l = 0; l < 2; ++l) v8[l][b8] = (ref[l] == 0 && col_zero) ? 0u : pv[l];
    }
    for (int l = 0; l < 2; ++l) {
      u32 row[2][4];
      for (int h = 0; h < 2; ++h) {
        row[h][0] = row[h][1] = v8[l][2 * h];
        row[h][2] = row[h][3] = v8[l][2 * h + 1];
      }
      u8* mv = reinterpret_cast<u8*>(&s.mv[l][0][0]);
      for (int y = 0; y < 4; ++y) std::memcpy(mv + 16 * y, row[y >> 1], 16);
    }
  }

  WpEntry weights(int r0, int r1) { return wp_entry(env_, r0, r1); }

  int cbf_luma_inc(int mb, int blk, bool intra) {
    auto cond = [&](int m, int nblk) -> int {
      if (m < 0) return intra ? 1 : 0;
      const MbState& n = nb_.at(m);
      if (n.kind == kIPcm) return 1;
      if (n.skip) return 0;
      if (!((n.cbp >> raster_b8(nblk)) & 1)) return 0;
      if (n.t8x8) return 1;
      return (n.cbf >> nblk) & 1;
    };
    const int bx = blk & 3, by = blk >> 2;
    const int a = bx > 0 ? cond(mb, blk - 1) : cond(nb_.mb_at(mb, -1, 0), blk + 3);
    const int b = by > 0 ? cond(mb, blk - 4) : cond(nb_.mb_at(mb, 0, -1), blk + 12);
    return a + 2 * b;
  }
  int cbf_dc_inc(int mb, int bit, bool intra) {
    auto cond = [&](int m) -> int {
      if (m < 0) return intra ? 1 : 0;
      const MbState& n = nb_.at(m);
      if (n.kind == kIPcm) return 1;
      if (bit == 0) return n.kind == kI16x16 ? (n.cbf_dc & 1) : 0;
      if (n.skip || (n.cbp >> 4) == 0) return 0;
      return (n.cbf_dc >> bit) & 1;
    };
    return cond(nb_.mb_at(mb, -1, 0)) + 2 * cond(nb_.mb_at(mb, 0, -1));
  }
  int cbf_cac_inc(int mb, int c, int b, bool intra) {
    auto cond = [&](int m, int nb2, bool cur) -> int {
      if (cur) return (nb_.at(mb).cbf_cac[c] >> nb2) & 1;
      if (m < 0) return intra ? 1 : 0;
      const MbState& n = nb_.at(m);
      if (n.kind == kIPcm) return 1;
// ... 482 lines not shown
```

csrc/vep/avc_recon.h:

```cpp
#pragma once

#include "common.h"

#if defined(__HIPCC__)
#include <hip/hip_runtime.h>
#define VEP_HD __host__ __device__ inline
#else
#define VEP_HD inline
#endif
#if defined(__HIP_DEVICE_COMPILE__)
#define VEP_CONST __constant__
#else
#define VEP_CONST
#endif

namespace vep::avc {

using i16 = int16_t;
using i8 = int8_t;

enum MbKind : u8 { kSkip = 0, kInter = 1, kI4x4 = 2, kI16x16 = 3, kIPcm = 4, kI8x8 = 5 };
VEP_HD bool is_intra(u8 k) { return k >= kI4x4; }
VEP_HD bool is_wave_intra(u8 k) { return k == kI4x4 || k == kI16x16 || k == kI8x8; }

constexpr u8 kMbT8x8 = 1;
constexpr u8 kMbL1 = 2;
constexpr u8 kMbWp = 4;
constexpr u8 kMbMv8x8 = 8;
constexpr u8 kMbMv16 = 16;

struct MbRec {
  u8 kind;
  u8 qp;
  u8 qpc;
  u8 qpc2;
  u8 i16_mode;
  u8 chroma_mode;
  u8 dbk;
  u8 flags;
  u16 nz;
  u16 luma_coded;
  i8 alpha_off;
  i8 beta_off;
  u16 slice;
  u16 chroma_coded;
  u16 pad1;
  u8 ref[4];
  u8 ref1[4];
  u32 coef;
  u32 mv;
  u8 i4[8];
  u32 res;
  u32 wp;
  u32 pad2;
};
static_assert(sizeof(MbRec) == 56, "MbRec layout");
constexpr u32 kNoRes = 0xFFFFFFFFu;

VEP_HD int mv_per_list(u8 flags) { return (flags & kMbMv16) ? 2 : ((flags & kMbMv8x8) ? 8 : 32); }
VEP_HD int byte_at(const u8* a, int i) {
  u32 w;
  __builtin_memcpy(&w, a, 4);
  return int((w >> (8 * i)) & 0xFFu);
}

VEP_HD int mv_sub(u8 flags, int list, int blk) {
  const int k = (flags & kMbMv16) ? 0 : ((flags & kMbMv8x8) ? 2 * (((blk >> 3) << 1) | ((blk & 3) >> 1)) : 2 * blk);
  return list * mv_per_list(flags) + k;
}

struct WpEntry {
  i16 w0[3], w1[3];
  i16 o[3];
  u8 lwd[3];
  u8 pad[11];
};
static_assert(sizeof(WpEntry) == 32, "WpEntry layout");

VEP_HD int wp_sample(int p0, int p1, bool has0, bool has1, const WpEntry* w, int c, int bd = 8) {
  if (!w) return has0 && has1 ? (p0 + p1 + 1) >> 1 : (has0 ? p0 : p1);
  const int lwd = w->lwd[c], mx = (1 << bd) - 1;
  if (has0 && has1) {
    const int v = ((p0 * w->w0[c] + p1 * w->w1[c] + (1 << lwd)) >> (lwd + 1)) + w->o[c];
    return v < 0 ? 0 : (v > mx ? mx : v);
  }
  const int p = has0 ? p0 : p1, ww = has0 ? w->w0[c] : w->w1[c];
  const int v = lwd >= 1 ? ((p * ww + (1 << (lwd - 1))) >> lwd) + w->o[c] : p * ww + w->o[c];
  return v < 0 ? 0 : (v > mx ? mx : v);
}

constexpr int kDenseCoefs = 512;
VEP_HD int coef_words(const MbRec& m) {
  return __builtin_popcount(u32(m.luma_coded)) + __builtin_popcount(u32(m.chroma_coded));
}
VEP_HD int coef_word_base(const MbRec& m, int j) {
  const u32 lc = m.luma_coded;
  const int nl = __builtin_popcount(lc);
  if (j >= nl) {
    u32 cc = m.chroma_coded;
    for (int k = j - nl; k > 0; --k) cc &= cc - 1;
    return 256 + 16 * __builtin_ctz(cc);
  }
  if (m.flags & kMbT8x8) {
    const u32 qm = (lc & 1u) | ((lc >> 1) & 2u) | ((lc >> 6) & 4u) | ((lc >> 7) & 8u);
    u32 q = qm;
    for (int k = j >> 2; k > 0; --k) q &= q - 1;
    return 64 * __builtin_ctz(q) + 16 * (j & 3);
  }
  u32 w = lc;
  for (int k = j; k > 0; --k) w &= w - 1;
// ... 737 lines not shown
  if (((mp.nz >> bp) & 1) || ((mq.nz >> bq) & 1)) return 2;
  const int p8 = ((bp >> 3) << 1) | ((bp & 3) >> 1), q8 = ((bq >> 3) << 1) | ((bq & 3) >> 1);
  const int p0 = word_byte(mp.ref, p8), p1 = (mp.flags & kMbL1) ? word_byte(mp.ref1, p8) : 0xFF;
  const int q0 = word_byte(mq.ref, q8), q1 = (mq.flags & kMbL1) ? word_byte(mq.ref1, q8) : 0xFF;
  const int np = (p0 != 0xFF) + (p1 != 0xFF), nq = (q0 != 0xFF) + (q1 != 0xFF);
  if (np != nq) return 1;
  const i16* pa = mv_p + mv_sub(mp.flags, 0, bp);
  const i16* pb = mv_p + mv_sub(mp.flags, 1, bp);
  const i16* qa = mv_q + mv_sub(mq.flags, 0, bq);
  const i16* qb = mv_q + mv_sub(mq.flags, 1, bq);
  if (np == 1) {
    const int rp = p0 != 0xFF ? p0 : p1, rq = q0 != 0xFF ? q0 : q1;
    if (rp != rq) return 1;
    return mv_far(p0 != 0xFF ? pa : pb, q0 != 0xFF ? qa : qb, ylim) ? 1 : 0;
  }
  if (!((p0 == q0 && p1 == q1) || (p0 == q1 && p1 == q0))) return 1;
  if (p0 != p1) {
    if (p0 == q0) return (mv_far(pa, qa, ylim) || mv_far(pb, qb, ylim)) ? 1 : 0;
    return (mv_far(pa, qb, ylim) || mv_far(pb, qa, ylim)) ? 1 : 0;
  }
  return ((mv_far(pa, qa, ylim) || mv_far(pb, qb, ylim)) && (mv_far(pa, qb, ylim) || mv_far(pb, qa, ylim))) ? 1 : 0;
}

VEP_HD int boundary_strength(BsSide mp, int bp, const i16* mv_p, BsSide mq, int bq,
                             const i16* mv_q, bool mb_edge, bool field = false, bool vertical = true) {
  if (is_intra(mp.kind) || is_intra(mq.kind)) return (mb_edge && (vertical || !field)) ? 4 : 3;
  if (field) return boundary_strength_mv(mp, bp, mv_p, mq, bq, mv_q, 2);
  return boundary_strength_mv(mp, bp, mv_p, mq, bq, mv_q, 4);
}

VEP_HD int boundary_strength(const MbRec& mp, int bp, const i16* mv_p, const MbRec& mq, int bq,
                             const i16* mv_q, bool mb_edge, bool field = false, bool vertical = true) {
  return boundary_strength(bs_side(mp), bp, mv_p, bs_side(mq), bq, mv_q, mb_edge, field, vertical);
}

struct EdgeParams {
  int alpha, beta;
  int tc0[3];
};

VEP_HD EdgeParams edge_params(int qp_p, int qp_q, int off_a, int off_b, int bd = 8) {
  const int qav = (qp_p + qp_q + 1) >> 1;
  const int ia = clip3(0, 51, qav + off_a), ib = clip3(0, 51, qav + off_b);
  const int s = bd - 8;
  return EdgeParams{kAlpha[ia] << s, kBeta[ib] << s, {kTc0[ia][0] << s, kTc0[ia][1] << s, kTc0[ia][2] << s}};
}

VEP_HD bool filter_samples(int* p, int* q, int bs, int alpha, int beta, int tc0, bool chroma, int bd = 8) {
  const int p0 = p[0], p1 = p[1], q0 = q[0], q1 = q[1];
  if (!(iabs(p0 - q0) < alpha && iabs(p1 - p0) < beta && iabs(q1 - q0) < beta)) return false;
  if (chroma) {
    if (bs < 4) {
      const int tc = tc0 + 1;
      const int d = clip3(-tc, tc, (((q0 - p0) << 2) + (p1 - q1) + 4) >> 3);
      p[0] = clip1(p0 + d, bd);
      q[0] = clip1(q0 - d, bd);
    } else {
      p[0] = (2 * p1 + p0 + q1 + 2) >> 2;
      q[0] = (2 * q1 + q0 + p1 + 2) >> 2;
    }
    return true;
  }
  const int p2 = p[2], q2 = q[2];
  const int ap = iabs(p2 - p0), aq = iabs(q2 - q0);
  if (bs < 4) {
    const int tc = tc0 + (ap < beta) + (aq < beta);
    const int d = clip3(-tc, tc, (((q0 - p0) << 2) + (p1 - q1) + 4) >> 3);
    p[0] = clip1(p0 + d, bd);
    q[0] = clip1(q0 - d, bd);
    if (ap < beta) p[1] = p1 + clip3(-tc0, tc0, (p2 + ((p0 + q0 + 1) >> 1) - (p1 << 1)) >> 1);
    if (aq < beta) q[1] = q1 + clip3(-tc0, tc0, (q2 + ((p0 + q0 + 1) >> 1) - (q1 << 1)) >> 1);
    return true;
  }
  const int p3 = p[3], q3 = q[3];
  const bool strong = iabs(p0 - q0) < ((alpha >> 2) + 2);
  if (ap < beta && strong) {
    p[0] = (p2 + 2 * p1 + 2 * p0 + 2 * q0 + q1 + 4) >> 3;
    p[1] = (p2 + p1 + p0 + q0 + 2) >> 2;
    p[2] = (2 * p3 + 3 * p2 + p1 + p0 + q0 + 4) >> 3;
  } else {
    p[0] = (2 * p1 + p0 + q1 + 2) >> 2;
  }
  if (aq < beta && strong) {
    q[0] = (p1 + 2 * p0 + 2 * q0 + 2 * q1 + q2 + 4) >> 3;
    q[1] = (p0 + q0 + q1 + q2 + 2) >> 2;
    q[2] = (2 * q3 + 3 * q2 + q1 + q0 + p0 + 4) >> 3;
  } else {
    q[0] = (2 * q1 + q0 + p1 + 2) >> 2;
  }
  return true;
}

VEP_HD bool filter_samples_u(int* p, int* q, int bs, int alpha, int beta, int tc0, bool chroma, int bd = 8) {
  const int p0 = p[0], p1 = p[1], p2 = p[2], p3 = p[3], q0 = q[0], q1 = q[1], q2 = q[2], q3 = q[3];
  if (!(iabs(p0 - q0) < alpha && iabs(p1 - p0) < beta && iabs(q1 - q0) < beta)) return false;
  const bool lp = !chroma && iabs(p2 - p0) < beta, lq = !chroma && iabs(q2 - q0) < beta;
  if (bs < 4) {
    const int tc = chroma ? tc0 + 1 : tc0 + int(lp) + int(lq);
    const int dl = clip3(-tc, tc, (((q0 - p0) << 2) + (p1 - q1) + 4) >> 3);
    p[0] = clip1(p0 + dl, bd);
    q[0] = clip1(q0 - dl, bd);
    if (lp) p[1] = p1 + clip3(-tc0, tc0, (p2 + ((p0 + q0 + 1) >> 1) - (p1 << 1)) >> 1);
    if (lq) q[1] = q1 + clip3(-tc0, tc0, (q2 + ((p0 + q0 + 1) >> 1) - (q1 << 1)) >> 1);
    return true;
  }
  const bool strong = iabs(p0 - q0) < ((alpha >> 2) + 2);
  if (lp && strong) {
    p[0] = (p2 + 2 * p1 + 2 * p0 + 2 * q0 + q1 + 4) >> 3;
    p[1] = (p2 + p1 + p0 + q0 + 2) >> 2;
    p[2] = (2 * p3 + 3 * p2 + p1 + p0 + q0 + 4) >> 3;
  } else {
    p[0] = (2 * p1 + p0 + q1 + 2) >> 2;
  }
  if (lq && strong) {
    q[0] = (p1 + 2 * p0 + 2 * q0 + 2 * q1 + q2 + 4) >> 3;
    q[1] = (p0 + q0 + q1 + q2 + 2) >> 2;
    q[2] = (2 * q3 + 3 * q2 + q1 + q0 + p0 + 4) >> 3;
  } else {
    q[0] = (2 * q1 + q0 + p1 + 2) >> 2;
  }
  return true;
}

template <typename Px>
VEP_HD void filter_line_t(Px* s, long step, int bs, int alpha, int beta, int tc0, bool chroma, int bd = 8) {
  const int n = chroma ? 2 : 4;
  int p[4] = {0, 0, 0, 0}, q[4] = {0, 0, 0, 0};
  for (int k = 0; k < n; ++k) {
    p[k] = s[-(k + 1) * step];
    q[k] = s[k * step];
  }
  if (!filter_samples(p, q, bs, alpha, beta, tc0, chroma, bd)) return;
  const int m = chroma ? 1 : 3;
  for (int k = 0; k < m; ++k) {
    s[-(k + 1) * step] = Px(p[k]);
    s[k * step] = Px(q[k]);
  }
}

template <typename Px>
VEP_HD void filter_line(Px* s, long step, int bs, const EdgeParams& e, bool chroma, int bd = 8) {
  filter_line_t(s, step, bs, e.alpha, e.beta, bs < 4 ? e.tc0[bs - 1] : 0, chroma, bd);
}

}
```

csrc/vep/gpu.h:

```cpp
#pragma once

#include <hip/hip_runtime.h>

#include <condition_variable>
#include <memory>
#include <mutex>

#include "common.h"

namespace vep::gpu {

#if defined(__HIP_DEVICE_COMPILE__) && defined(VEP_KERNEL_SOURCE)
#define VEP_DEV __attribute__((address_space(1)))
#else
#define VEP_DEV
#endif

#define VEP_HIP(expr)                                                                    \
  do {                                                                                   \
    hipError_t _e = (expr);                                                              \
    if (_e != hipSuccess)                                                                \
      throw ::vep::Error(std::string("HIP error ") + hipGetErrorString(_e) + " at " +     \
                         __FILE__ + ":" + std::to_string(__LINE__) + ": " #expr);        \
  } while (0)

int device_count();
bool rocdecode_available();

struct DecodeDesc {
  VEP_DEV u8* y;
  VEP_DEV u8* uv;
  VEP_DEV u8* bgr;
  const VEP_DEV u32* mask;
  const VEP_DEV u32* prefix;
  const VEP_DEV u32* offsets;
  const VEP_DEV u8* payload;
  const VEP_DEV u64* ptrs;
  i32 wmbs, hmbs;
  i32 out_w, out_h;
  i32 crop_left, crop_top;
  i32 tile_begin;
  i32 tiles_x;
  i32 chk_lo, chk_hi;
  u32 chk_pat;
  VEP_DEV u32* err;
};
constexpr int kTileMbW = 8, kTileMbH = 2;
inline int tiles_for(int wmbs, int hmbs) {
  return ((wmbs + kTileMbW - 1) / kTileMbW) * ((hmbs + kTileMbH - 1) / kTileMbH);
}

void launch_decode_convert(const DecodeDesc* d_descs, int n, int total_tiles, hipStream_t s);
void launch_decode_convert_one(const DecodeDesc& d, hipStream_t s);

struct SurfaceBgrDesc {
  const VEP_DEV u8* y;
  const VEP_DEV u8* uv;
  VEP_DEV u8* bgr;
  i32 pitch;
  i32 coded_w, coded_h;
  i32 bit_depth;
// ... 46 lines not shown
  i32 xg_h;
  u32 epoch;
  i32 npu, pu_begin;
  i32 blk_begin;
  u32 nap_max;
  u32 pad_;
};
inline size_t hevc_xg_words(int stride, int h) { return size_t(stride) * size_t(h) * 3 / 4; }
struct HevcTuRange {
  i32 desc, first, count, begin;
};
void launch_hevc_mc(const HevcDesc* d_descs, int n, int total_pus, hipStream_t s);
void launch_hevc_tu(const HevcDesc* d_descs, const HevcTuRange* d_ranges, int nranges, int base, int count,
                    hipStream_t s);
void launch_hevc_tu_queue(const HevcDesc* d_descs, const HevcTuRange* d_ranges, int nranges, int base, int count,
                          u32* ctr, bool persistent, hipStream_t s);
void launch_hevc_tu_pics(const HevcDesc* d_descs, const HevcTuRange* d_pics, int npics, hipStream_t s);
void launch_hevc_deblock(const HevcDesc* d_descs, int n, int total_blocks, int dir, hipStream_t s);
void launch_hevc_sao(const HevcDesc* d_descs, int n, int total_blocks, hipStream_t s);
void launch_narrow(const void* y, const void* uv, u8* y8, u8* uv8, int w, int h, int bd, int cf, hipStream_t s);
struct WeaveDesc {
  const VEP_DEV u8* y;
  const VEP_DEV u8* uv;
  VEP_DEV u8* y8;
  VEP_DEV u8* uv8;
  i32 pitch, height;
};
void launch_weave(const WeaveDesc* d_descs, int n, int max_pitch, int max_height, hipStream_t s);

struct AvcDesc {
  const VEP_DEV void* mbs;
  const VEP_DEV i16* coefs;
  const VEP_DEV i16* mvs;
  const VEP_DEV void* wps;
  VEP_DEV u8* y;
  VEP_DEV u8* uv;
  u64 slot_y, slot_uv;
  i32 wmbs, hmbs;
  i32 target;
  i32 constrained;
  i32 mb_begin;
  i32 field;
  VEP_DEV u32* err;
  VEP_DEV void* dbk;
  VEP_DEV i16* res;
  VEP_DEV u64* prof;
  i32 bd;
  i32 qp_bias, qpc_bias;
  i32 cf;
  u32 ncoef, nres;
  i32 intra_mbs;
  i32 deblock;
  VEP_DEV u64* xg;
};
constexpr int kAvcProfSlots = 20;
constexpr int kAvcResSamples = 512;
struct AvcDbkInfo {
  u32 bs[4];
  u8 alpha[9], beta[9];
  u8 tc0[9][3];
  u8 any;
  u8 pad[1];
};
static_assert(sizeof(AvcDbkInfo) == 64, "AvcDbkInfo layout");
constexpr int kAvcDbkWgRows = 8;
constexpr int kAvcXgWords = 24;
inline int avc_dbk_groups(int hmbs) { return (hmbs + kAvcDbkWgRows - 1) / kAvcDbkWgRows; }
inline size_t avc_xg_bytes(int wmbs, int hmbs) {
  return size_t(avc_dbk_groups(hmbs) - 1) * size_t(wmbs) * kAvcXgWords * sizeof(u64);
}
constexpr int kAvcMaxRows = 512;
constexpr int kAvcMaxCols = 512;
void launch_avc_inter(const AvcDesc* d_descs, int n, int total_mbs, hipStream_t s);
void launch_avc_intra(const AvcDesc* d_descs, int n, int max_hmbs, hipStream_t s);
void launch_avc_bs(const AvcDesc* d_descs, int n, int total_mbs, hipStream_t s);
void launch_avc_deblock(const AvcDesc* d_descs, int n, int max_hmbs, hipStream_t s, int packed = 1);
void launch_avc_hbd(const AvcDesc* d_descs, int n, bool intra, bool dbk, int variants, hipStream_t s);

struct JpegDesc {
  const VEP_DEV u8* bgr;
  i32 w, h, quality;
  i32 mcus_x, mcus;
  i32 intervals;
  VEP_DEV i16* coefs;
  VEP_DEV u8* seg;
  VEP_DEV u32* len;
  VEP_DEV u32* off;
  VEP_DEV u8* out;
  u32 out_cap;
  VEP_DEV u32* status;
};
void launch_jpeg_transform(const JpegDesc& d, hipStream_t s);
void launch_jpeg_entropy(const JpegDesc& d, hipStream_t s);
void launch_jpeg_scan(const JpegDesc& d, hipStream_t s);
void launch_jpeg_gather(const JpegDesc& d, hipStream_t s);

class JpegPool {
 public:
  JpegPool();
  ~JpegPool();
  JpegPool(const JpegPool&) = delete;
  JpegPool& operator=(const JpegPool&) = delete;
  bool encode(const u8* d_bgr, int w, int h, int quality, hipStream_t s, std::string& out);
  static constexpr int kScratch = 4;

 private:
  struct Scratch;
  Scratch* acquire();
  void release(Scratch* sc);
  std::mutex mu_;
  std::condition_variable cv_;
  std::vector<std::unique_ptr<Scratch>> all_;
  std::vector<Scratch*> free_;
};

struct ScaleDesc {
  const VEP_DEV u8* src;
  VEP_DEV u8* dst;
  u32 src_pitch, dst_pitch;
  i32 sw, sh;
  i32 dx, dy, ow, oh;
  i32 cx, cy, cw, ch;
};
static_assert(sizeof(ScaleDesc) == 64, "ScaleDesc layout");
void check_scale(const ScaleDesc& d, int canvas_w, int canvas_h);
// ... 111 lines not shown
```

csrc/vep/gpu_avc.hip:

```cpp
#define VEP_KERNEL_SOURCE 1
#include "avc_recon.h"
#include "gpu.h"

namespace vep::gpu {

using avc::MbRec;
using avc::kDenseCoefs;

namespace {

constexpr int kIntraWaves = kAvcDbkWgRows;
constexpr int kIntraXgWords = 8;
constexpr int kIntraLine = 32;
constexpr int kIntraLineCols = 240;
constexpr u32 kSpinLimit = 1u << 24;

__device__ inline const MbRec& rec(const AvcDesc& d, int mb) {
  return static_cast<const MbRec*>(d.mbs)[mb];
}


__device__ inline void wave_sync() {
  __builtin_amdgcn_fence(__ATOMIC_RELEASE, "wavefront");
  __builtin_amdgcn_wave_barrier();
// ... 123 lines not shown
    if (s0 != 0xFF) {
      const i16* v0 = mvb + avc::mv_sub(m.flags, 0, blk);
      p0 = avc::luma_qpel(yref(s0), pitch, wpx, hpx, mx * 16 + x + (v0[0] >> 2),
                          my * 16 + y + (v0[1] >> 2), v0[0] & 3, v0[1] & 3, bd);
    }
    if (s1 != 0xFF) {
      const i16* v1 = mvb + avc::mv_sub(m.flags, 1, blk);
      p1 = avc::luma_qpel(yref(s1), pitch, wpx, hpx, mx * 16 + x + (v1[0] >> 2),
                          my * 16 + y + (v1[1] >> 2), v1[0] & 3, v1[1] & 3, bd);
    }
    v[k] = avc::wp_sample(p0, p1, s0 != 0xFF, s1 != 0xFF, wpp ? wpp + b8 : nullptr, 0, bd);
  }
  if (m.luma_coded | m.chroma_coded) expand_coefs_wave(d, m, lane, D);
  if (t8) luma8_residual(D, m, lane, T);
#pragma unroll
  for (int k = 0; k < 4; ++k) {
    const int y = y0 + 4 * k, blk = k * 4 + (x >> 2);
    int o = v[k];
    if (t8) o += T[y * 16 + x];
    else if ((m.luma_coded >> blk) & 1) o += avc::idct4x4_at(D + 16 * blk, y & 3, x & 3);
    ty[size_t(my * 16 + y) * pitch + mx * 16 + x] = P(avc::clip1(o, bd));
  }
  int u[NCL];
  const int chp = CF == 2 ? hpx : hpx / 2;
#pragma unroll
  for (int k = 0; k < NCL; ++k) {
    const int t = lane + 64 * k, cc = t / CS, cq = t % CS, cx = cq & 7, cy = cq >> 3;
    const int ly = CF == 2 ? cy : 2 * cy;
    const int r = (ly >> 2) * 4 + (cx >> 1), b8 = ((ly >> 3) << 1) | (cx >> 2);
    const int s0 = avc::byte_at(m.ref, b8), s1 = l1 ? avc::byte_at(m.ref1, b8) : 0xFF;
    int p0 = 0, p1 = 0, ix, fx, iy, fy;
    if (s0 != 0xFF) {
      const i16* v0 = mvb + avc::mv_sub(m.flags, 0, r);
      const int vy = v0[1] + (d.field ? 2 * ((d.field == 2) - (s0 & 1)) : 0);
      avc::chroma_mv(v0[0], vy, CF, ix, fx, iy, fy);
      p0 = avc::chroma_epel(uvref(s0), pitch, wpx / 2, chp, cc, mx * 8 + cx + ix, my * CH + cy + iy, fx, fy);
    }
    if (s1 != 0xFF) {
      const i16* v1 = mvb + avc::mv_sub(m.flags, 1, r);
      const int vy = v1[1] + (d.field ? 2 * ((d.field == 2) - (s1 & 1)) : 0);
      avc::chroma_mv(v1[0], vy, CF, ix, fx, iy, fy);
      p1 = avc::chroma_epel(uvref(s1), pitch, wpx / 2, chp, cc, mx * 8 + cx + ix, my * CH + cy + iy, fx, fy);
    }
    u[k] = avc::wp_sample(p0, p1, s0 != 0xFF, s1 != 0xFF, wpp ? wpp + b8 : nullptr, 1 + cc, bd);
  }
#pragma unroll
  for (int k = 0; k < NCL; ++k) {
    const int t = lane + 64 * k, cc = t / CS, cq = t % CS, cx = cq & 7, cy = cq >> 3;
    const int kb = cc * NB + (cy >> 2) * 2 + (cx >> 2);
    int o = u[k];
    if ((m.chroma_coded >> kb) & 1) o += avc::idct4x4_at(D + 256 + 16 * kb, cy & 3, cx & 3);
    tuv[size_t(my * CH + cy) * pitch + (mx * 8 + cx) * 2 + cc] = P(avc::clip1(o, bd));
  }
}

__global__ __launch_bounds__(256) void avc_inter_kernel(const AvcDesc* __restrict__ descs, int n,
                                                         int total) {
  __shared__ int lres[4][kT8Ints];
  __shared__ alignas(16) i16 lcoef[4][kDenseCoefs];
  const int wv = int(threadIdx.x) >> 6;
  const int g = __builtin_amdgcn_readfirstlane(int(blockIdx.x) * 4 + wv);
  if (g >= total) return;
  int lo = 0, hi = n - 1;
  while (lo < hi) {
    const int mid = (lo + hi + 1) >> 1;
    if (descs[mid].mb_begin <= g) lo = mid;
    else hi = mid - 1;
  }
  const AvcDesc d = descs[lo];
  const int mb = g - d.mb_begin;
  const MbRec m = rec(d, mb);
  const int lane = int(threadIdx.x) & 63;
  const int x = lane & 15, y0 = lane >> 4;
  int* T = lres[wv];
  const bool t8 = (m.flags & avc::kMbT8x8) && m.luma_coded;
  if (avc::is_wave_intra(m.kind)) {
    const int row = mb / d.wmbs;
    if (lane < kIntraXgWords && row % kAvcDbkWgRows == kAvcDbkWgRows - 1 && row + 1 < d.hmbs)
      d.xg[(size_t(row / kAvcDbkWgRows) * d.wmbs + mb % d.wmbs) * kAvcXgWords + lane] = 0;
    if (m.res == avc::kNoRes) return;
    if ((d.bd > 8 || d.cf == 2) && m.res >= d.nres) {
      atomicOr(d.err, 0x8000u);
      return;
    }
    i16* r = d.res + size_t(m.res) * kAvcResSamples;
    i16* D = lcoef[wv];
    expand_coefs_wave(d, m, lane, D);
    if (t8) luma8_residual(D, m, lane, T);
#pragma unroll
    for (int k = 0; k < 4; ++k) {
      const int y = y0 + 4 * k, blk = k * 4 + (x >> 2);
      int v;
      if (t8) v = T[y * 16 + x];
      else v = (m.luma_coded >> blk) & 1 ? avc::idct4x4_at(D + 16 * blk, y & 3, x & 3) : 0;
      r[y * 16 + x] = i16(v);
    }
    const int ncs = d.cf == 2 ? 128 : 64, nb = d.cf == 2 ? 8 : 4;
    for (int k = 0; k < 2 * ncs / 64; ++k) {
      const int t = lane + 64 * k, cc = t / ncs, cq = t % ncs, cx = cq & 7, cy = cq >> 3;
      const int kb = cc * nb + (cy >> 2) * 2 + (cx >> 2);
      r[256 + t] = i16((m.chroma_coded >> kb) & 1 ? avc::idct4x4_at(D + 256 + 16 * kb, cy & 3, cx & 3) : 0);
    }
    return;
  }
  if (m.kind != avc::kSkip && m.kind != avc::kInter && m.kind != avc::kIPcm) return;
  if (d.cf == 2) {
// ... 953 lines not shown
        st4(&L.carry[l * 4], w_carry);
      } else {
        L.ccarry[cc][ck * 2] = cr0;
        L.ccarry[cc][ck * 2 + 1] = cr1;
      }
    }
    if (x == W - 1) {
      __builtin_amdgcn_fence(__ATOMIC_RELEASE, "workgroup", "local");
      if (l == 0 && act)
        __hip_atomic_store(&sync.progress[lrow], u32(W + 1), __ATOMIC_RELAXED, __HIP_MEMORY_SCOPE_WORKGROUP);
    }
    wave_sync();
    cur = nxt;
    if (d.prof) {
      const u64 t7 = clock64();
      acc[0] += (t1 - t0) + (t4 - t3);
      acc[1] += (t2 - t1) + (t5 - t4);
      acc[2] += (t3 - t2) + (t6 - t5);
      acc[3] += t7 - t6;
      acc[4] += u64(__popcll(__ballot(act) & 0x100000001ull));
    }
  }
  if (d.prof && lane == 0)
    for (int k = 0; k < 5; ++k) atomicAdd(&d.prof[6 + k], acc[k]);
}

__global__ __launch_bounds__(256) void weave_kernel(const WeaveDesc* __restrict__ descs) {
  const WeaveDesc d = descs[blockIdx.y];
  const u8* __restrict__ y = d.y;
  const u8* __restrict__ uv = d.uv;
  u8* __restrict__ y8 = d.y8;
  u8* __restrict__ uv8 = d.uv8;
  const int pitch = d.pitch, h = d.height;
  const int per_row = pitch / 16;
  const size_t g = size_t(blockIdx.x) * 256 + threadIdx.x, total = size_t(per_row) * size_t(h + h / 2);
  if (g >= total) return;
  const int row = int(g / size_t(per_row)), col = int(g % size_t(per_row)) * 16;
  const bool luma = row < h;
  const int r = luma ? row : row - h, fh = luma ? h / 2 : h / 4;
  const u8* src = (luma ? y : uv) + (size_t(r & 1) * size_t(fh) + size_t(r >> 1)) * size_t(pitch) + size_t(col);
  u8* dst = (luma ? y8 : uv8) + size_t(r) * size_t(pitch) + size_t(col);
  *reinterpret_cast<uint4*>(dst) = *reinterpret_cast<const uint4*>(src);
}

}

void launch_weave(const WeaveDesc* d_descs, int n, int max_pitch, int max_height, hipStream_t s) {
  if (n <= 0 || max_pitch <= 0 || max_height <= 0) return;
  const size_t lanes = size_t(max_pitch / 16) * size_t(max_height + max_height / 2);
  hipLaunchKernelGGL(weave_kernel, dim3(unsigned((lanes + 255) / 256), unsigned(n)), dim3(256), 0, s, d_descs);
  VEP_HIP(hipGetLastError());
}

void launch_avc_inter(const AvcDesc* d_descs, int n, int total_mbs, hipStream_t s) {
  if (n <= 0 || total_mbs <= 0) return;
  hipLaunchKernelGGL(avc_inter_kernel, dim3(unsigned((total_mbs + 3) / 4)), dim3(256), 0, s, d_descs, n,
                     total_mbs);
  VEP_HIP(hipGetLastError());
}

void launch_avc_intra(const AvcDesc* d_descs, int n, int max_hmbs, hipStream_t s) {
  if (n <= 0 || max_hmbs <= 0) return;
  const int groups = avc_dbk_groups(max_hmbs);
  const unsigned blocks = unsigned((n + 7) / 8) * unsigned(groups) * 8u;
  hipLaunchKernelGGL(avc_intra_kernel, dim3(blocks), dim3(64 * kIntraWaves), 0, s, d_descs, n, groups);
  VEP_HIP(hipGetLastError());
}

void launch_avc_bs(const AvcDesc* d_descs, int n, int total_mbs, hipStream_t s) {
  if (n <= 0 || total_mbs <= 0) return;
  hipLaunchKernelGGL(avc_bs_kernel, dim3(unsigned((total_mbs + 255) / 256)), dim3(256), 0, s, d_descs,
                     n, total_mbs);
  VEP_HIP(hipGetLastError());
}

void launch_avc_deblock(const AvcDesc* d_descs, int n, int max_hmbs, hipStream_t s, int packed) {
  if (n <= 0 || max_hmbs <= 0) return;
  const int groups = (max_hmbs + kDbkRows - 1) / kDbkRows;
  const unsigned blocks = unsigned((n + 7) / 8) * unsigned(groups) * 8u;
  hipLaunchKernelGGL(avc_deblock_kernel, dim3(blocks), dim3(64 * kDbkWaves), 0, s, d_descs, n, groups, packed);
  VEP_HIP(hipGetLastError());
}

}
```

csrc/vep/runtime.cpp:

```cpp
#include "runtime.h"

#include <algorithm>
#include <array>
#include <chrono>
#include <cmath>
#include <csignal>
#include <cstdio>
#include <map>
#include <thread>

#include "color.h"
#include "jpeg.h"
#include "scale.h"
#include "trace.h"

namespace vep {


Device::Device(int id) : id_(id) {
  if (id_ >= 0) {
    int n = gpu::device_count();
    VEP_CHECK(id_ < n, "GPU " + std::to_string(id_) + " not present (" + std::to_string(n) +
                           " visible)");
    bind();
// ... 1252 lines not shown
    const int s = u.slot[size_t(mb)];
    const u32 g = u.slot_seg[size_t(s)];
    ptrs[k++] = reinterpret_cast<u64>(seg_dev[g] + (u.block(s) - u.segs[g].base));
  }
  u32 run = 0;
  for (int w = 0; w < words; ++w) {
    prefix[w] = run;
    run += u32(__builtin_popcount(mask[w]));
  }
}

constexpr size_t kPackChunk = size_t(1) << 20;

}

void Worker::launch_gpu(Lane& ln, Stage& st) {
  const hipStream_t cs = ln.stream;
  std::vector<DecodeJob>& jobs = st.jobs;
  const int n = int(jobs.size());
  const bool direct = direct_reads_;
  const size_t off_desc = 0;
  const size_t off_lb = al(sizeof(gpu::DecodeDesc) * size_t(n));
  size_t nchunks = 0;
  auto chunks_of = [](size_t len) { return (len + gpu::kGatherChunk - 1) / gpu::kGatherChunk; };
  if (!direct)
    for (const auto& j : jobs)
      for (const auto& sg : j.upd.segs) nchunks += chunks_of(sg.len);
  auto pinned = [](const void* p, size_t len) {
    return len > 0 && hostmem::device_address(static_cast<const u8*>(p), len) != nullptr;
  };
  const size_t off_wv = off_lb + al(sizeof(gpu::LetterboxDesc) * size_t(n));
  size_t need = off_wv + al(sizeof(gpu::WeaveDesc) * size_t(n));
  struct HistOut {
    int round, job, out;
  };
  std::vector<HistOut> hist;
  for (int i = 0; i < n; ++i)
    for (size_t k = 0; k < jobs[size_t(i)].outputs.size(); ++k)
      if (jobs[size_t(i)].outputs[k].ring_slot >= 0) hist.push_back({jobs[size_t(i)].outputs[k].released_by, i, int(k)});
  const size_t off_hist = need;
  need += al(sizeof(gpu::SurfaceBgrDesc) * hist.size());
  std::vector<size_t> mask_off(static_cast<size_t>(n)), pay_off(static_cast<size_t>(n));
  std::vector<std::vector<size_t>> seg_off(static_cast<size_t>(n));
  auto words_of = [&](int i) { return size_t(jobs[size_t(i)].upd.mbs() + 31) / 32; };
  const size_t ent = direct ? sizeof(u64) : sizeof(u32);
  for (int i = 0; i < n; ++i) {
    mask_off[size_t(i)] = need;
    need += 2 * al(words_of(i) * sizeof(u32), 16) +
            al(size_t(jobs[size_t(i)].upd.nslots) * ent, 16);
  }
  struct AvcPic {
    const avc::Picture* p;
    int job;
    size_t off_mbs, off_coef, off_mv, off_wp, off_dbk, off_res, off_xg;
  };
  std::vector<AvcPic> apics;
  int rounds = 0;
  for (int i = 0; i < n; ++i) rounds = std::max(rounds, int(jobs[size_t(i)].avc.size()));
  std::vector<size_t> off_round(static_cast<size_t>(rounds));
  std::vector<std::vector<int>> round_pics(static_cast<size_t>(rounds));
  for (int r = 0; r < rounds; ++r) {
    for (int i = 0; i < n; ++i) {
      const auto& v = jobs[size_t(i)].avc;
      if (int(v.size()) <= r) continue;
      const avc::Picture& p = *v[size_t(r)];
      VEP_CHECK(p.hmbs <= gpu::kAvcMaxRows && p.wmbs <= gpu::kAvcMaxCols,
                "picture too large for the wavefront kernels");
      VEP_CHECK(p.wmbs * 16 == jobs[size_t(i)].pic.coded_width &&
                    p.hmbs * 16 * (p.structure ? 2 : 1) == jobs[size_t(i)].pic.coded_height,
                "picture size differs from the camera's surfaces");
      AvcPic a{&p, i, 0, 0, 0, 0, 0, 0, 0};
      auto put = [&](const void* src, size_t bytes) {
        const size_t o = need;
        need += al(bytes);
        if (pinned(src, bytes)) nchunks += chunks_of(bytes);
        return o;
      };
      a.off_mbs = put(p.mbs.data(), p.mbs.size() * sizeof(avc::MbRec));
      a.off_coef = put(p.coefs.data(), p.coefs.size() * sizeof(i16));
      a.off_mv = put(p.mvs.data(), p.mvs.size() * sizeof(i16));
      a.off_wp = put(p.wps.data(), p.wps.size() * sizeof(avc::WpEntry));
      round_pics[size_t(r)].push_back(int(apics.size()));
      apics.push_back(a);
    }
    off_round[size_t(r)] = need;
    need += al(round_pics[size_t(r)].size() * sizeof(gpu::AvcDesc));
  }
  struct HevcPic {
    const hevc::GpuPicture* p;
    int job;
    size_t off_pu, off_tu, off_coef, off_pcm, off_bsv, off_bsh, off_qp, off_pcmmap, off_cslice, off_slices, off_sao;
    size_t off_wp, off_ctile;
  };
  std::vector<HevcPic> hpics;
  int hrounds = 0;
  for (int i = 0; i < n; ++i) hrounds = std::max(hrounds, int(jobs[size_t(i)].hevc.size()));
  std::vector<size_t> off_hround(static_cast<size_t>(hrounds)), off_hranges(static_cast<size_t>(hrounds));
  std::vector<std::vector<int>> hround_pics(static_cast<size_t>(hrounds));
  std::vector<std::vector<gpu::HevcTuRange>> hranges(static_cast<size_t>(hrounds));
  std::vector<std::array<int, 4>> hwork(static_cast<size_t>(hrounds), std::array<int, 4>{0, 0, 0, 0});
  std::vector<size_t> off_hctr(static_cast<size_t>(hrounds)), off_hpicq(static_cast<size_t>(hrounds));
  std::vector<std::vector<gpu::HevcTuRange>> hpicq(static_cast<size_t>(hrounds));
  std::vector<std::vector<std::array<int, 2>>> hlevels(static_cast<size_t>(hrounds));
  std::vector<std::vector<std::array<int, 2>>> hwindows(static_cast<size_t>(hrounds));
  for (int r = 0; r < hrounds; ++r) {
    int maxl = 0;
    for (int i = 0; i < n; ++i) {
      const auto& v = jobs[size_t(i)].hevc;
      if (int(v.size()) <= r) continue;
      const hevc::GpuPicture& p = *v[size_t(r)];
      VEP_CHECK(((p.width + 15) & ~15) == jobs[size_t(i)].pic.coded_width &&
                    ((p.height + 15) & ~15) == jobs[size_t(i)].pic.coded_height,
                "picture size differs from the camera's surfaces");
      HevcPic a{&p, i, 0, 0, 0, 0, 0, 0, 0, 0, 0, 0, 0, 0, 0};
      auto put = [&](size_t bytes) {
        const size_t o = need;
        need += al(std::max<size_t>(bytes, 16));
        return o;
      };
      a.off_pu = put(p.pus.size() * sizeof(hevc::GpuPu));
      a.off_tu = put(p.tus.size() * sizeof(hevc::GpuTu));
      a.off_coef = put(p.coefs.size() * sizeof(i16));
      a.off_pcm = put(p.pcm.size());
      a.off_bsv = put(p.bs_v.size());
      a.off_bsh = put(p.bs_h.size());
      a.off_qp = put(p.qp.size());
      a.off_pcmmap = put(p.pcm_map.size());
      a.off_cslice = put(p.ctb_slice.size() * sizeof(u16));
      a.off_slices = put(p.slices.size() * sizeof(hevc::GpuSlice));
      a.off_sao = put(p.sao_params.size() * sizeof(hevc::GpuSao));
      a.off_wp = put(p.wp.size() * sizeof(hevc::GpuWp));
      a.off_ctile = put(p.ctb_tile.size() * sizeof(u16));
      maxl = std::max(maxl, int(p.level_begin.size()) - 1);
      hround_pics[size_t(r)].push_back(int(hpics.size()));
// ... 45 lines not shown
    off_hpicq[size_t(r)] = need;
    need += al(std::max<size_t>(hpicq[size_t(r)].size(), 1) * sizeof(gpu::HevcTuRange));
  }
  const size_t off_gather = need;
  need += al(sizeof(gpu::GatherChunk) * std::max<size_t>(nchunks, 1));
  need = al(need);
  const size_t header_bytes = need;
  for (int i = 0; i < n; ++i) {
    pay_off[size_t(i)] = need;
    size_t rel = 0;
    for (const auto& sg : jobs[size_t(i)].upd.segs) {
      seg_off[size_t(i)].push_back(rel);
      rel += al(sg.len, 16);
    }
    need += rel;
  }
  need = al(need);
  for (AvcPic& a : apics) {
    a.off_dbk = need;
    need += al(size_t(a.p->nmbs()) * sizeof(gpu::AvcDbkInfo));
    a.off_res = need;
    need += al(size_t(a.p->intra_res) * gpu::kAvcResSamples * sizeof(i16));
    a.off_xg = need;
    need += al(gpu::avc_xg_bytes(a.p->wmbs, a.p->hmbs));
  }
  need = al(need);
  if (need > st.cap) {
    if (st.h) hostmem::unregister_range(st.h);
    dev_.free(st.d);
    dev_.free_pinned(st.h);
    st.cap = std::max(need + need / 2, size_t(4) << 20);
    st.h = static_cast<u8*>(dev_.alloc_pinned(st.cap));
    st.d = static_cast<u8*>(dev_.alloc(st.cap));
    void* hd_ptr = nullptr;
    if (hipHostGetDevicePointer(&hd_ptr, st.h, 0) != hipSuccess) hd_ptr = st.h;
    hostmem::register_range(st.h, st.cap, static_cast<u8*>(hd_ptr));
  }
  auto mask_ptr = [&](u8* base, int i) { return reinterpret_cast<u32*>(base + mask_off[size_t(i)]); };
  auto prefix_ptr = [&](u8* base, int i) {
    return reinterpret_cast<u32*>(base + mask_off[size_t(i)] + al(words_of(i) * sizeof(u32), 16));
  };
  auto table_ptr = [&](u8* base, int i) {
    return base + mask_off[size_t(i)] + 2 * al(words_of(i) * sizeof(u32), 16);
  };
  struct CopyTask {
    const u8* src;
    u8* dst;
    size_t len;
  };
  std::vector<CopyTask> tasks;
  auto* gc = reinterpret_cast<gpu::GatherChunk*>(st.h + off_gather);
  size_t ng = 0;
  for (const AvcPic& a : apics) {
    auto add = [&](const void* src, size_t len, size_t off) {
      if (pinned(src, len)) {
        const u8* dv = hostmem::device_address(static_cast<const u8*>(src), len);
        for (size_t o = 0; o < len; o += gpu::kGatherChunk)
          gc[ng++] = {dv + o, st.d + off + o, u32(std::min<size_t>(gpu::kGatherChunk, len - o)), 0};
        records_gathered_ += u64(len);
        return;
      }
      for (size_t o = 0; o < len; o += kPackChunk)
        tasks.push_back({static_cast<const u8*>(src) + o, st.h + off + o, std::min(kPackChunk, len - o)});
    };
    add(a.p->mbs.data(), a.p->mbs.size() * sizeof(avc::MbRec), a.off_mbs);
    add(a.p->coefs.data(), a.p->coefs.size() * sizeof(i16), a.off_coef);
    add(a.p->mvs.data(), a.p->mvs.size() * sizeof(i16), a.off_mv);
    add(a.p->wps.data(), a.p->wps.size() * sizeof(avc::WpEntry), a.off_wp);
  }
  for (const HevcPic& a : hpics) {
    auto add = [&](const void* src, size_t len, size_t off) {
      for (size_t o = 0; o < len; o += kPackChunk)
        tasks.push_back({static_cast<const u8*>(src) + o, st.h + off + o, std::min(kPackChunk, len - o)});
    };
    const hevc::GpuPicture& p = *a.p;
    add(p.pus.data(), p.pus.size() * sizeof(hevc::GpuPu), a.off_pu);
    add(p.tus.data(), p.tus.size() * sizeof(hevc::GpuTu), a.off_tu);
    add(p.coefs.data(), p.coefs.size() * sizeof(i16), a.off_coef);
    add(p.pcm.data(), p.pcm.size(), a.off_pcm);
    add(p.bs_v.data(), p.bs_v.size(), a.off_bsv);
    add(p.bs_h.data(), p.bs_h.size(), a.off_bsh);
    add(p.qp.data(), p.qp.size(), a.off_qp);
    add(p.pcm_map.data(), p.pcm_map.size(), a.off_pcmmap);
    add(p.ctb_slice.data(), p.ctb_slice.size() * sizeof(u16), a.off_cslice);
    add(p.slices.data(), p.slices.size() * sizeof(hevc::GpuSlice), a.off_slices);
    add(p.sao_params.data(), p.sao_params.size() * sizeof(hevc::GpuSao), a.off_sao);
    add(p.wp.data(), p.wp.size() * sizeof(hevc::GpuWp), a.off_wp);
    add(p.ctb_tile.data(), p.ctb_tile.size() * sizeof(u16), a.off_ctile);
  }
  std::vector<std::vector<const u8*>> seg_dev(static_cast<size_t>(n));
  for (int i = 0; i < n; ++i) {
    const auto& segs = jobs[size_t(i)].upd.segs;
    for (size_t g = 0; g < segs.size(); ++g) {
      const size_t dst_off = pay_off[size_t(i)] + seg_off[size_t(i)][g];
      const u8* src = hostmem::device_address(segs[g].base, segs[g].len);
      if (!src) {
        for (size_t o = 0; o < segs[g].len; o += kPackChunk)
          tasks.push_back({segs[g].base + o, st.h + dst_off + o,
                           std::min(kPackChunk, segs[g].len - o)});
        src = hostmem::device_address(st.h + dst_off, segs[g].len);
        VEP_CHECK(src, "staging buffer is not registered");
        pinned_bytes_staged_ += u64(segs[g].len);
      } else {
        pinned_bytes_inplace_ += u64(segs[g].len);
      }
      seg_dev[size_t(i)].push_back(src);
      if (!direct)
        for (size_t o = 0; o < segs[g].len; o += gpu::kGatherChunk)
          gc[ng++] = {src + o, st.d + dst_off + o,
                      u32(std::min<size_t>(gpu::kGatherChunk, segs[g].len - o)), 0};
    }
  }
  VEP_CHECK(ng == nchunks, "gather chunk count mismatch");
  auto index = [&](int i) {
    if (direct)
      build_index_ptrs(jobs[size_t(i)].upd, seg_dev[size_t(i)], mask_ptr(st.h, i),
                       prefix_ptr(st.h, i), reinterpret_cast<u64*>(table_ptr(st.h, i)));
    else
      build_index(jobs[size_t(i)].upd, seg_off[size_t(i)], mask_ptr(st.h, i), prefix_ptr(st.h, i),
                  reinterpret_cast<u32*>(table_ptr(st.h, i)));
  };
// ... 132 lines not shown
      d.chroma_format = sf.cf;
      d.crop_left = o.pic.crop_left;
      d.crop_top = o.pic.crop_top;
      d.out_w = o.pic.width;
      d.out_h = o.pic.height;
      d.tile_begin = hr[2];
      gpu::check_surface_bgr(d);
      VEP_CHECK(o.slot < sf.slots && d.out_w == c->ring_->width() && d.out_h == c->ring_->height(),
                "history output does not match the camera's surfaces");
      hr[1] += 1;
      hr[2] += gpu::tiles_for(sf.wmbs, sf.hmbs);
    }
  }
  auto convert_history = [&](int r) {
    const std::array<int, 3>& hr = hist_round[size_t(r)];
    if (hr[1] > 0)
      gpu::launch_surface_to_bgr(reinterpret_cast<const gpu::SurfaceBgrDesc*>(st.d + off_hist) + hr[0], hr[1], hr[2], cs);
  };
  for (int r = 0; r < rounds; ++r) {
    auto* ad = reinterpret_cast<gpu::AvcDesc*>(st.h + off_round[size_t(r)]);
    int mbs = 0;
    for (size_t k = 0; k < round_pics[size_t(r)].size(); ++k) {
      const AvcPic& a = apics[size_t(round_pics[size_t(r)][k])];
      const Camera* c = cams_[size_t(jobs[size_t(a.job)].cam)].get();
      gpu::AvcDesc& g = ad[k];
      g.mbs = st.d + a.off_mbs;
      g.coefs = reinterpret_cast<const i16*>(st.d + a.off_coef);
      g.mvs = reinterpret_cast<const i16*>(st.d + a.off_mv);
      g.wps = st.d + a.off_wp;
      g.y = c->surface.y;
      g.uv = c->surface.uv;
      const size_t per = a.p->structure ? 2 : 1;
      g.slot_y = c->surface.slot_y() / per;
      g.slot_uv = c->surface.slot_uv() / per;
      g.wmbs = a.p->wmbs;
      g.hmbs = a.p->hmbs;
      g.target = a.p->target;
      g.constrained = a.p->constrained_intra ? 1 : 0;
      g.mb_begin = mbs;
      g.field = a.p->structure;
      g.err = const_cast<u32*>(st.err_dev) + a.job;
      g.dbk = st.d + a.off_dbk;
      g.res = reinterpret_cast<i16*>(st.d + a.off_res);
      g.xg = reinterpret_cast<u64*>(st.d + a.off_xg);
      g.prof = avc_prof_;
      g.bd = a.p->bd;
      g.qp_bias = a.p->qp_bias;
      g.qpc_bias = a.p->qpc_bias;
      g.cf = a.p->cf;
      g.ncoef = u32(a.p->coefs.size());
      g.nres = u32(a.p->intra_res);
      g.intra_mbs = a.p->intra_mbs;
      g.deblock = a.p->deblock ? 1 : 0;
      VEP_CHECK(c->surface.bd == a.p->bd && c->surface.cf == a.p->cf,
                "H.264: picture bit depth / chroma format differs from the camera's surfaces");
      mbs += a.p->nmbs();
    }
  }
  std::vector<std::array<int, 2>> hround_work(static_cast<size_t>(hrounds));
  for (int r = 0; r < hrounds; ++r) {
    auto* hd2 = reinterpret_cast<gpu::HevcDesc*>(st.h + off_hround[size_t(r)]);
    int pus = 0, blks = 0;
    for (size_t k = 0; k < hround_pics[size_t(r)].size(); ++k) {
      const HevcPic& a = hpics[size_t(hround_pics[size_t(r)][k])];
      const hevc::GpuPicture& p = *a.p;
      const DecodeJob& j = jobs[size_t(a.job)];
      const Camera* c = cams_[size_t(j.cam)].get();
      gpu::HevcDesc& g = hd2[k];
      g = gpu::HevcDesc{};
      g.y = c->surface.y;
      g.uv = c->surface.uv;
      g.slot_y = c->surface.slot_y();
      g.slot_uv = c->surface.slot_uv();
      g.stride = c->surface.wmbs * 16;
      g.width = p.width;
      g.height = p.height;
      g.log2ctb = p.log2ctb;
      g.wctb = p.wctb;
      g.hctb = p.hctb;
      g.target = p.target;
      g.cb_qp_offset = p.cb_qp_offset;
      g.cr_qp_offset = p.cr_qp_offset;
      g.flags = (p.deblock ? 1 : 0) | (p.sao ? 2 : 0) | (p.pcm_nofilter ? 4 : 0) | (p.tiles_block_sao ? 8 : 0) |
                (p.wide() ? gpu::kHevcWide : 0);
      VEP_CHECK(c->surface.bps == (p.wide() ? 2 : 1), "HEVC: picture bit depth differs from the camera's surfaces");
      g.bd_y = p.bd_y;
      g.bd_c = p.bd_c;
      g.pus = st.d + a.off_pu;
      g.tus = st.d + a.off_tu;
      g.coefs = reinterpret_cast<const i16*>(st.d + a.off_coef);
      g.pcm = st.d + a.off_pcm;
      g.bs_v = st.d + a.off_bsv;
      g.bs_h = st.d + a.off_bsh;
      g.qp = reinterpret_cast<const signed char*>(st.d + a.off_qp);
      g.pcm_map = st.d + a.off_pcmmap;
      g.ctb_slice = reinterpret_cast<const u16*>(st.d + a.off_cslice);
      g.slices = st.d + a.off_slices;
      g.sao = st.d + a.off_sao;
      g.wp = st.d + a.off_wp;
      g.ctb_tile = reinterpret_cast<const u16*>(st.d + a.off_ctile);
      const size_t scratch = size_t(j.hevc_slots);
      VEP_CHECK(c->surface.slots > j.hevc_slots, "camera surfaces lack the SAO scratch slot");
      g.sao_y = c->surface.y + scratch * c->surface.slot_y();
      g.sao_uv = c->surface.uv + scratch * c->surface.slot_uv();
      g.err = const_cast<u32*>(st.err_dev) + a.job;
      {
// ... 7 lines not shown
          sf.hevc_epoch = 0;
        }
        if (++sf.hevc_epoch == 0) {
          VEP_HIP(hipMemset(sf.hevc_xg, 0, words * sizeof(u64)));
          sf.hevc_epoch = 1;
        }
        g.xg = hevc_tu_window_ == 0 ? nullptr : sf.hevc_xg;
        g.xg_h = sf.hmbs * 16;
        g.epoch = sf.hevc_epoch;
        g.nap_max = hevc_tu_nap_;
      }
      g.npu = int(p.pus.size());
      g.pu_begin = pus;
      g.blk_begin = blks;
      pus += g.npu;
      blks += p.w4() * p.h4();
    }
    hround_work[size_t(r)] = {pus, blks};
    auto* hr = reinterpret_cast<gpu::HevcTuRange*>(st.h + off_hranges[size_t(r)]);
    for (size_t k = 0; k < hranges[size_t(r)].size(); ++k) hr[k] = hranges[size_t(r)][k];
    std::memset(st.h + off_hctr[size_t(r)], 0, std::max<size_t>(hwindows[size_t(r)].size(), 1) * sizeof(u32));
    if (!hpicq[size_t(r)].empty())
      std::memcpy(st.h + off_hpicq[size_t(r)], hpicq[size_t(r)].data(), hpicq[size_t(r)].size() * sizeof(gpu::HevcTuRange));
  }
  if (ln.copy) {
    VEP_HIP(hipMemcpyAsync(st.d, st.h, header_bytes, hipMemcpyHostToDevice, ln.copy));
    if (nchunks)
      gpu::launch_gather(reinterpret_cast<const gpu::GatherChunk*>(st.d + off_gather),
                         int(nchunks), ln.copy);
    VEP_HIP(hipEventRecord(st.copied, ln.copy));
    VEP_HIP(hipStreamWaitEvent(cs, st.copied, 0));
    VEP_HIP(hipEventRecord(st.e0, cs));
  } else if (lanes_.size() > 1) {
    VEP_HIP(hipEventRecord(st.e0, cs));
    VEP_HIP(hipMemcpyAsync(st.d, st.h, header_bytes, hipMemcpyHostToDevice, cs));
    if (nchunks)
      gpu::launch_gather(reinterpret_cast<const gpu::GatherChunk*>(st.d + off_gather),
                         int(nchunks), cs);
  } else {
    VEP_HIP(hipMemcpyAsync(st.d, st.h, header_bytes, hipMemcpyHostToDevice, copy_stream_));
    if (nchunks)
      gpu::launch_gather(reinterpret_cast<const gpu::GatherChunk*>(st.d + off_gather),
                         int(nchunks), copy_stream_);
    VEP_HIP(hipEventRecord(st.copied, copy_stream_));
    VEP_HIP(hipStreamWaitEvent(cs, st.copied, 0));
    VEP_HIP(hipEventRecord(st.e0, cs));
  }
  for (int r = 0; r < rounds; ++r) {
    const auto* ad = reinterpret_cast<const gpu::AvcDesc*>(st.d + off_round[size_t(r)]);
    const int np = int(round_pics[size_t(r)].size());
    int mbs = 0;
    bool intra = false, dbk = false, narrow = false;
    int variants = 0;
    int max_h = 0;
    for (int k : round_pics[size_t(r)]) {
      mbs += apics[size_t(k)].p->nmbs();
      max_h = std::max(max_h, apics[size_t(k)].p->hmbs);
      intra |= apics[size_t(k)].p->intra_mbs > 0;
      dbk |= apics[size_t(k)].p->deblock;
      const avc::Picture& ap = *apics[size_t(k)].p;
      if (ap.bd > 8 || ap.cf == 2) variants |= ap.cf != 2 ? 1 : (ap.bd > 8 ? 4 : 2);
      else narrow = true;
    }
    gpu::launch_avc_inter(ad, np, mbs, cs);
    if (intra && narrow) gpu::launch_avc_intra(ad, np, max_h, cs);
    if (dbk) {
      gpu::launch_avc_bs(ad, np, mbs, cs);
      if (narrow) gpu::launch_avc_deblock(ad, np, max_h, cs, dbk_packed_);
    }
    if (variants) gpu::launch_avc_hbd(ad, np, intra, dbk, variants, cs);
    convert_history(r);
  }
  for (int r = 0; r < hrounds; ++r) {
    const auto* hd2 = reinterpret_cast<const gpu::HevcDesc*>(st.d + off_hround[size_t(r)]);
    const auto* hr = reinterpret_cast<const gpu::HevcTuRange*>(st.d + off_hranges[size_t(r)]);
    const int np = int(hround_pics[size_t(r)].size());
    bool dbk = false, sao = false;
    for (int k : hround_pics[size_t(r)]) {
      dbk |= hpics[size_t(k)].p->deblock;
      sao |= hpics[size_t(k)].p->sao;
    }
    gpu::launch_hevc_mc(hd2, np, hround_work[size_t(r)][0], cs);
    const auto& hw = hwork[size_t(r)];
    gpu::launch_hevc_tu(hd2, hr, hw[0], 0, hw[1], cs);
    if (hevc_tu_window_ < 0) {
      gpu::launch_hevc_tu_pics(hd2, reinterpret_cast<const gpu::HevcTuRange*>(st.d + off_hpicq[size_t(r)]),
                               int(hpicq[size_t(r)].size()), cs);
    } else if (hevc_tu_window_ == 0) {
      for (const auto& lv : hlevels[size_t(r)]) gpu::launch_hevc_tu(hd2, hr + hw[0], hw[2], lv[0], lv[1], cs);
    } else {
      auto* ctr = reinterpret_cast<u32*>(st.d + off_hctr[size_t(r)]);
      const bool persistent = hevc_tu_window_ >= kAllLevels;
      for (size_t k = 0; k < hwindows[size_t(r)].size(); ++k)
        gpu::launch_hevc_tu_queue(hd2, hr + hw[0], hw[2], hwindows[size_t(r)][k][0], hwindows[size_t(r)][k][1],
                                  ctr + k, persistent, cs);
    }
    if (dbk) {
      gpu::launch_hevc_deblock(hd2, np, hround_work[size_t(r)][1], 0, cs);
      gpu::launch_hevc_deblock(hd2, np, hround_work[size_t(r)][1], 1, cs);
    }
    if (sao) gpu::launch_hevc_sao(hd2, np, hround_work[size_t(r)][1], cs);
    convert_history(rounds + r);
  }
  for (int i = 0; i < n; ++i) {
    const DecodeJob& j = jobs[size_t(i)];
    if (!j.ext) continue;
    const Camera* c = cams_[size_t(j.cam)].get();
    const vcn::Frame& f = *j.ext;
    const size_t pitch = size_t(c->surface.wmbs) * 16;
    VEP_CHECK(size_t(f.width) <= pitch && f.height <= c->surface.hmbs * 16, "VCN picture exceeds the camera surface");
    VEP_HIP(hipMemcpy2DAsync(c->surface.y, pitch, f.y, f.pitch_y, size_t(f.width), size_t(f.height),
                             hipMemcpyDefault, cs));
    VEP_HIP(hipMemcpy2DAsync(c->surface.uv, pitch, f.uv, f.pitch_uv, size_t(f.width), size_t(f.height / 2),
                             hipMemcpyDefault, cs));
  }
  gpu::launch_weave(reinterpret_cast<const gpu::WeaveDesc*>(st.d + off_wv), nweave, weave_pitch, weave_h, cs);
// ... 22 lines not shown
  }
  VEP_HIP(hipEventRecord(st.e1, cs));
  add_time(&Timers::enqueue, double(mono_us() - t_enq0));
}

void Worker::run_cpu(std::vector<DecodeJob>& jobs, std::vector<int>& slots,
                     std::vector<u32>& err) {
  err.assign(jobs.size(), 0);
  std::vector<std::vector<size_t>> groups;
  std::map<int, size_t> of;
  for (size_t i = 0; i < jobs.size(); ++i) {
    auto it = of.find(jobs[i].cam);
    if (it == of.end()) {
      of[jobs[i].cam] = groups.size();
      groups.push_back({i});
    } else {
      groups[it->second].push_back(i);
    }
  }
  auto run = [&](int g) {
    for (size_t i : groups[size_t(g)]) run_cpu_job(jobs, slots, err, i);
  };
  if (cpu_pool_ && groups.size() > 1) cpu_pool_->parallel_for(int(groups.size()), run);
  else
    for (int g = 0; g < int(groups.size()); ++g) run(g);
}

void Worker::run_cpu_job(std::vector<DecodeJob>& jobs, std::vector<int>& slots, std::vector<u32>& err, size_t i) {
  {
    Camera& c = *cams_[size_t(jobs[i].cam)];
    const PictureInfo& pi = jobs[i].pic;
    for (int sl = pi.spec_lo; sl < pi.spec_hi && !err[i]; ++sl) {
      const u8* b = jobs[i].upd.block(sl);
      err[i] = (b[-2] != 0x0D || b[-1] != 0x00) ? 1u : 0u;
    }
    if (err[i]) return;
    if (jobs[i].ext) {
      const vcn::Frame& f = *jobs[i].ext;
      HostSurface& hs = c.surface.host[0];
      VEP_CHECK(f.width <= hs.coded_w && f.height <= hs.coded_h, "VCN picture exceeds the camera surface");
      for (int r = 0; r < f.height; ++r)
        std::memcpy(&hs.y[size_t(r) * size_t(hs.coded_w)], f.y + size_t(r) * f.pitch_y, size_t(f.width));
      for (int r = 0; r < f.height / 2; ++r)
        std::memcpy(&hs.uv[size_t(r) * size_t(hs.coded_w)], f.uv + size_t(r) * f.pitch_uv, size_t(f.width));
    } else if (jobs[i].general()) {
      auto convert_history = [&](size_t k) {
        for (const JobOutput& o : jobs[i].outputs)
          if (o.ring_slot >= 0 && size_t(o.released_by) == k)
            cpu_nv12_to_bgr(c.surface.host[size_t(o.slot)], o.pic.crop_left, o.pic.crop_top, o.pic.width, o.pic.height,
                            c.ring_->slot_ptr(o.ring_slot));
      };
      for (size_t k = 0; k < jobs[i].avc.size(); ++k) {
        const auto& pic = jobs[i].avc[k];
        if (!pic->structure) {
          avc::cpu_reconstruct(*pic, c.surface.host);
          convert_history(k);
          continue;
        }
        auto& F = c.surface.fields;
        if (F.size() < size_t(pic->dpb_slots)) F.resize(size_t(pic->dpb_slots));
        for (auto& h : F)
          if (h.coded_w != pic->wmbs * 16 || h.coded_h != pic->hmbs * 16 || h.bd != pic->bd || h.cf != pic->cf)
            h.alloc(pic->wmbs * 16, pic->hmbs * 16, pic->bd, pic->cf);
        avc::cpu_reconstruct(*pic, F);
      }
      for (size_t k = 0; k < jobs[i].hevc.size(); ++k) {
        hevc::cpu_execute(*jobs[i].hevc[k], c.surface.host);
        convert_history(k);
      }
    } else {
      cpu_apply_update(jobs[i].upd, c.surface.host[0]);
    }
    if (!jobs[i].has_output()) return;
    HostSurface narrow;
    HostSurface woven;
    if (jobs[i].out_fields) {
      const size_t t = size_t(jobs[i].target());
      VEP_CHECK(2 * t + 1 < c.surface.fields.size(), "field pair output without its fields");
      avc::weave_fields(c.surface.fields[2 * t], c.surface.fields[2 * t + 1], woven);
    }
    const HostSurface& out = jobs[i].out_fields ? woven : c.surface.host[size_t(jobs[i].target())];
    const bool conv = out.wide() || out.cf == 2;
    if (conv) narrow_surface(out, narrow);
    const HostSurface& src = conv ? narrow : out;
    cpu_nv12_to_bgr(src, jobs[i].pic.crop_left, jobs[i].pic.crop_top,
                    jobs[i].pic.width, jobs[i].pic.height, c.ring_->slot_ptr(slots[i]));
    if (opt_.ref_copies) {
      const size_t n = size_t(jobs[i].pic.width) * size_t(jobs[i].pic.height) * 3;
      std::vector<u8> bytes(c.ring_->slot_ptr(slots[i]), c.ring_->slot_ptr(slots[i]) + n);
      FrameMeta m{};
      m.width = jobs[i].pic.width;
      m.height = jobs[i].pic.height;
      m.pts = jobs[i].meta.pts;
      const auto pre_suf = encode_video_frame(m, n, c.name());
      std::string msg;
      msg.reserve(pre_suf.first.size() + n + pre_suf.second.size());
      msg += pre_suf.first;
      msg.append(reinterpret_cast<const char*>(bytes.data()), n);
      msg += pre_suf.second;
      ref_copy_bytes_.fetch_add(msg.size(), std::memory_order_relaxed);
    }
    if (opt_.letterbox_size > 0) {
      gpu::LetterboxDesc l{};
      const size_t S = size_t(opt_.letterbox_size);
      l.src_w = jobs[i].pic.width;
      l.src_h = jobs[i].pic.height;
// ... 1259 lines not shown
```

Before: 8398.

## Encode runs of uniform skipped H.264 macroblocks compactly and expand them on GPU

The parser now collapses consecutive P/B-skip macroblocks within a row that share an identical record and motion into a single SkipRun descriptor instead of writing a full MbRec and motion entry per macroblock. Gather chunks that are fully covered by runs are left out of the host-to-device upload, and a new GPU kernel expands the runs into the record and MV arrays before the inter kernel runs. CPU paths (fallback reconstruct, validation, parallel slices) call expand_runs. This is meant to reduce parser store bandwidth and PCIe/gather traffic on skip-heavy streams, at the cost of an extra kernel launch per round, added bookkeeping, and more complexity.

New measurement: 8465, median of 3. No clear change (+0.8%).

```diff
diff --git a/csrc/bindings.cpp b/csrc/bindings.cpp
--- a/csrc/bindings.cpp
+++ b/csrc/bindings.cpp
@@ -189,6 +189,7 @@
         for (auto& h : slots)
           if (h.coded_w != pic->wmbs * 16 || h.coded_h != pic->hmbs * 16 || h.bd != pic->bd || h.cf != pic->cf)
             h.alloc(pic->wmbs * 16, pic->hmbs * 16, pic->bd, pic->cf);
+        pic->expand_runs();
         avc::cpu_reconstruct(*pic, slots);
         coded = pic->info.coded_mbs;
         pictures.push_back(pic->info);
@@ -963,6 +964,7 @@
       auto p = dec.parse(*au);
       if (!p) continue;
       ++pics;
+      p->expand_runs();
       mbs += p->mbs.size();
       coefs += p->coefs.size();
       mvs += p->mvs.size();
@@ -2133,6 +2135,153 @@
     return py::make_tuple(d.nw, d.nh, d.pad_x, d.pad_y);
   }, py::arg("src_w"), py::arg("src_h"), py::arg("size"), py::arg("even") = false);
 
+  m.def("avc_set_skip_runs", [](int mode) { avc::set_skip_runs(mode); }, py::arg("mode"));
+  m.def("avc_skip_runs_enabled", [] { return avc::skip_runs_enabled(); });
+  m.def("avc_parse_records",
+        [](const std::vector<std::shared_ptr<AccessUnit>>& aus, int skip_runs, bool expand, bool reconstruct,
+           int parallel) {
+          struct Out {
+            std::string mbs, mvs, coefs, wps;
+            std::vector<i32> col;
+            bool has_col = false;
+            int runs = 0, run_mbs = 0, inter = 0, intra = 0, intra_res = 0, wmbs = 0, hmbs = 0;
+            char type = 0;
+            u64 par = 0;
+          };
+          std::vector<Out> outs;
+          {
+            py::gil_scoped_release nogil;
+            struct Restore {
+              ~Restore() { avc::set_skip_runs(-1); }
+            } restore;
+            avc::set_skip_runs(skip_runs);
+            avc::Decoder dec;
+            dec.keep_col = true;
+            if (parallel >= 0) dec.set_parallel_slices(parallel != 0);
+            std::vector<HostSurface> slots;
+            for (const auto& au : aus) {
+              size_t nal = 0;
+              do {
+                avc::PicturePtr p = dec.parse(*au, 0, &nal);
+                Out o;
+                o.runs = int(p->runs.size());
+                o.run_mbs = p->run_mbs;
+                if (expand) p->expand_runs();
+                if (reconstruct) {
+                  if (slots.size() < size_t(p->dpb_slots)) slots.resize(size_t(p->dpb_slots));
+                  for (auto& h : slots)
+                    if (h.coded_w != p->wmbs * 16 || h.coded_h != p->hmbs * 16 || h.bd != p->bd || h.cf != p->cf)
+                      h.alloc(p->wmbs * 16, p->hmbs * 16, p->bd, p->cf);
+                  avc::cpu_reconstruct(*p, slots);
+                }
+                if (expand) {
+                  o.mbs.assign(reinterpret_cast<const char*>(p->mbs.data()), p->mbs.size() * sizeof(avc::MbRec));
+                  o.mvs.assign(reinterpret_cast<const char*>(p->mvs.data()), p->mvs.size() * sizeof(i16));
+                }
+                o.coefs.assign(reinterpret_cast<const char*>(p->coefs.data()), p->coefs.size() * sizeof(i16));
+                o.wps.assign(reinterpret_cast<const char*>(p->wps.data()), p->wps.size() * sizeof(avc::WpEntry));
+                if (dec.last_col) {
+                  o.has_col = true;
+                  for (const auto& b : dec.last_col->b) {
+                    o.col.push_back(b.mv[0]);
+                    o.col.push_back(b.mv[1]);
+                    o.col.push_back(i32(b.pid));
+                    o.col.push_back(b.ref);
+                  }
+                }
+                o.inter = p->inter_mbs;
+                o.intra = p->intra_mbs;
+                o.intra_res = p->intra_res;
+                o.wmbs = p->wmbs;
+                o.hmbs = p->hmbs;
+                o.type = p->info.pict_type;
+                o.par = dec.parallel_slices_run();
+                outs.push_back(std::move(o));
+              } while (nal < au->nals.size());
+            }
+          }
+          py::list l;
+          for (const Out& o : outs) {
+            py::dict d;
+            d["mbs"] = py::bytes(o.mbs);
+            d["mvs"] = py::bytes(o.mvs);
+            d["coefs"] = py::bytes(o.coefs);
+            d["wps"] = py::bytes(o.wps);
+            if (o.has_col) {
+              py::array_t<i32> c({py::ssize_t(o.col.size() / 4), py::ssize_t(4)});
+              std::memcpy(c.mutable_data(), o.col.data(), o.col.size() * sizeof(i32));
+              d["col"] = c;
+            } else {
+              d["col"] = py::none();
+            }
+            d["runs"] = o.runs;
+            d["run_mbs"] = o.run_mbs;
+            d["inter_mbs"] = o.inter;
+            d["intra_mbs"] = o.intra;
+            d["intra_res"] = o.intra_res;
+            d["wmbs"] = o.wmbs;
+            d["hmbs"] = o.hmbs;
+            d["type"] = std::string(1, o.type);
+            d["parallel_slices_run"] = o.par;
+            l.append(d);
+          }
+          return l;
+        },
+        py::arg("aus"), py::arg("skip_runs") = -1, py::arg("expand") = true, py::arg("reconstruct") = false,
+        py::arg("parallel") = -1);
+  m.def("avc_expand_runs",
+        [](py::bytes runs_bytes, int nmbs, int nmv, int fill, bool on_gpu) {
+          const std::string rb = runs_bytes;
+          VEP_CHECK(rb.size() % sizeof(avc::SkipRun) == 0 && nmbs >= 0 && nmv >= 0, "avc_expand_runs: bad arguments");
+          avc::Picture pic;
+          pic.wmbs = std::max(nmbs, 1);
+          pic.hmbs = 1;
+          avc::MbRec frec;
+          std::memset(&frec, fill, sizeof frec);
+          i16 fmv;
+          std::memset(&fmv, fill, sizeof fmv);
+          pic.mbs.assign(size_t(nmbs), frec);
+          pic.mvs.assign(size_t(nmv), fmv);
+          const size_t n = rb.size() / sizeof(avc::SkipRun);
+          if (n) pic.runs.append(reinterpret_cast<const avc::SkipRun*>(rb.data()), n);
+          gpu::check_skip_runs(pic.runs.data(), n, size_t(nmbs), size_t(nmv));
+          const size_t bm = size_t(nmbs) * sizeof(avc::MbRec), bv = size_t(nmv) * sizeof(i16);
+          if (!on_gpu) {
+            pic.expand_runs();
+          } else {
+            auto al = [](size_t b) { return (b + 255) & ~size_t(255); };
+            const size_t o_mv = al(bm), o_runs = o_mv + al(bv), o_desc = o_runs + al(rb.size()), total = o_desc + 256;
+            std::vector<u8> h(total, u8(fill));
+            std::memcpy(h.data(), pic.mbs.data(), bm);
+            std::memcpy(h.data() + o_mv, pic.mvs.data(), bv);
+            std::memcpy(h.data() + o_runs, rb.data(), rb.size());
+            void* dv = nullptr;
+            VEP_HIP(hipMalloc(&dv, total));
+            u8* d = static_cast<u8*>(dv);
+            gpu::AvcDesc desc{};
+            desc.mbs = d;
+            desc.mvs = reinterpret_cast<const i16*>(d + o_mv);
+            desc.runs = d + o_runs;
+            desc.nruns = u32(n);
+            std::memcpy(h.data() + o_desc, &desc, sizeof desc);
+            try {
+              VEP_HIP(hipMemcpy(d, h.data(), total, hipMemcpyHostToDevice));
+              gpu::launch_avc_expand_runs(reinterpret_cast<const gpu::AvcDesc*>(d + o_desc), 1, int(n), nullptr);
+              VEP_HIP(hipDeviceSynchronize());
+              VEP_HIP(hipMemcpy(h.data(), d, total, hipMemcpyDeviceToHost));
+            } catch (...) {
+              (void)hipFree(dv);
+              throw;
+            }
+            (void)hipFree(dv);
+            std::memcpy(static_cast<void*>(pic.mbs.data()), h.data(), bm);
+            std::memcpy(pic.mvs.data(), h.data() + o_mv, bv);
+          }
+          return py::make_tuple(py::bytes(reinterpret_cast<const char*>(pic.mbs.data()), bm),
+                                py::bytes(reinterpret_cast<const char*>(pic.mvs.data()), bv));
+        },
+        py::arg("runs"), py::arg("nmbs"), py::arg("nmv"), py::arg("fill") = 0xA5, py::arg("gpu") = false);
+
   bind_net(m);
   bind_mux(m);
   bind_hevc(m);
diff --git a/csrc/vep/avc.cpp b/csrc/vep/avc.cpp
--- a/csrc/vep/avc.cpp
+++ b/csrc/vep/avc.cpp
@@ -4,6 +4,7 @@
 
 #include <algorithm>
 #include <array>
+#include <atomic>
 
 #include "avc_cavlc.h"
 #include "avc_internal.h"
@@ -1294,8 +1295,11 @@
     auto mbs = std::move(p.mbs);
     auto coefs = std::move(p.coefs), mvs = std::move(p.mvs);
     auto wps = std::move(p.wps);
+    auto runs = std::move(p.runs);
     std::vector<OutFrame> outputs = std::move(p.outputs);
     p = Picture{};
+    runs.clear();
+    p.runs = std::move(runs);
     coefs.clear();
     mvs.clear();
     wps.clear();
@@ -1509,6 +1513,7 @@
   }
   VEP_CHECK(got, "access unit has no slice");
   (void)act_pps;
+  if (keep_col) last_col = col_built;
   std::vector<u8> covered;
   if (par) {
     const int W = pic->wmbs, H = pic->hmbs;
@@ -1523,6 +1528,10 @@
       sh.coefs.clear();
       sh.mvs.clear();
       sh.wps.clear();
+      sh.runs.clear();
+      sh.run_mbs = 0;
+      sh.runs_expanded = false;
+      sh.open_run.open = false;
       sh.intra_mbs = sh.intra_res = sh.inter_mbs = 0;
       sh.deblock = false;
       sh.target = pic->target;
@@ -1537,6 +1546,7 @@
       u.colb.set_uids(&u.uids);
       sh.colb = col_target ? &u.colb : nullptr;
       parse_slice_data(u.nb, sh, u.sh, *u.sps, *u.pps, u.rbsp.data(), u.rbsp.size(), u.bitpos, u.slice_idx, u.list);
+      sh.expand_runs();
 #if defined(__x86_64__)
       _mm_sfence();
 #endif
@@ -1623,6 +1633,7 @@
     if (first.has_mmco5()) pic->poc = 0;
     bump(*pic, out_of(*pic), boundary, boundary && (hard_flush || reorder_cur_ == 0));
   }
+  if (missing) pic->expand_runs();
   if (missing || par) validate(*pic);
   else validate_picture(*pic);
   return pic;
@@ -1676,6 +1687,7 @@
   env.scaling = h264::resolve_scaling(sps, pps);
   env.field = sh.field_pic;
   decode_slice_generic(nb, pic, env, data, n, bitpos);
+  pic.flush_run();
 }
 
 static inline void validate_mb(const Picture& p, const MbRec& m, bool written = false) {
@@ -1761,6 +1773,7 @@
 
 void validate(const Picture& p) {
   validate_picture(p);
+  p.records();
   for (const MbRec& m : p.mbs) validate_mb(p, m);
 }
 
@@ -1785,21 +1798,30 @@
   for (int k = 0; k < per; ++k) out[k] = ColMotion::Blk{{0, 0}, 0u, i8(-1)};
 }
 
+void ColBuild::corner_entries(const MbState& st, ColMotion::Blk out[4]) const {
+  static constexpr u8 kCorner[4] = {0, 3, 12, 15};
+  for (int k = 0; k < 4; ++k) {
+    const int l = st.ref[0][k] >= 0 ? 0 : 1;
+    const int ri = st.ref[l][k];
+    out[k] = ri < 0 ? ColMotion::Blk{{0, 0}, 0u, i8(-1)}
+                    : ColMotion::Blk{{st.mv[l][kCorner[k]][0], st.mv[l][kCorner[k]][1]}, uid_tab[l][ri & 31], i8(ri)};
+  }
+}
+
+void ColBuild::fill(int mb0, int count, const void* entries) {
+  ColMotion::Blk* out = &col->b[size_t(mb0) * 4];
+  for (int i = 0; i < count; ++i) stream_words(out + 4 * i, entries, 4 * sizeof(ColMotion::Blk));
+}
+
 void ColBuild::store(int mb, const MbState& st) {
   if (is_intra(st.kind) || !uids) {
     none(mb);
     return;
   }
-  static constexpr u8 kCorner[4] = {0, 3, 12, 15};
   const auto& lu = *uids;
   if (col->corners) {
     ColMotion::Blk out[4];
-    for (int k = 0; k < 4; ++k) {
-      const int l = st.ref[0][k] >= 0 ? 0 : 1;
-      const int ri = st.ref[l][k];
-      out[k] = ri < 0 ? ColMotion::Blk{{0, 0}, 0u, i8(-1)}
-                      : ColMotion::Blk{{st.mv[l][kCorner[k]][0], st.mv[l][kCorner[k]][1]}, uid_tab[l][ri & 31], i8(ri)};
-    }
+    corner_entries(st, out);
     stream_words(&col->b[size_t(mb) * 4], out, sizeof out);
     return;
   }
@@ -2059,10 +2081,15 @@
 #endif
 }
 
-static inline void store_motion(Picture& pic, MbRec& m, const MbState& s) {
+static inline u32 mb_motion_uniformity(const MbRec& m, const MbState& s) {
   const int nl = (m.flags & kMbL1) ? 2 : 1;
   u32 u = 3;
   for (int l = 0; l < nl; ++l) u &= motion_uniformity(&s.mv[l][0][0]);
+  return u;
+}
+
+static inline void store_motion(Picture& pic, MbRec& m, const MbState& s, u32 u) {
+  const int nl = (m.flags & kMbL1) ? 2 : 1;
   m.flags |= (u & 1) ? kMbMv16 : ((u & 2) ? kMbMv8x8 : 0);
   m.mv = u32(pic.mvs.size());
   const int per = (u & 1) ? 2 : ((u & 2) ? 8 : 32);
@@ -2087,29 +2114,121 @@
   stream_words(dst, &m, sizeof(MbRec));
 }
 
+namespace {
+std::atomic<int> g_skip_runs{-1};
+}
+bool skip_runs_enabled() {
+  static const bool env = [] {
+    const char* e = std::getenv("VEP_SKIP_RUNS");
+    return !(e && e[0] == '0');
+  }();
+  const int o = g_skip_runs.load(std::memory_order_relaxed);
+  return o < 0 ? env : o != 0;
+}
+void set_skip_runs(int mode) { g_skip_runs.store(mode < 0 ? -1 : (mode ? 1 : 0), std::memory_order_relaxed); }
+
+void Picture::flush_run() {
+  OpenRun& o = open_run;
+  if (!o.open) return;
+  o.open = false;
+  static_assert(sizeof(SkipRun) % 8 == 0, "8-byte words");
+  if (o.r.count == 1) {
+    stream_words(&mbs[size_t(o.r.mb0)], &o.r.rec, sizeof(MbRec));
+    std::memcpy(mvs.data() + o.r.mv0, o.r.mv, o.r.mv_stride * sizeof(i16));
+    if (colb) colb->fill(int(o.r.mb0), 1, o.col);
+    return;
+  }
+  stream_words(runs.extend(1), &o.r, sizeof(SkipRun));
+  run_mbs += int(o.r.count);
+  if (colb) colb->fill(int(o.r.mb0), int(o.r.count), o.col);
+}
+
+void Picture::expand_runs() const {
+  if (runs.empty() || runs_expanded) return;
+  MbRec* recs = const_cast<MbRec*>(mbs.data());
+  i16* pool = const_cast<i16*>(mvs.data());
+  for (const SkipRun& r : runs) {
+    VEP_CHECK(r.count >= 1 && u64(r.mb0) + r.count <= mbs.size() && (r.mv_stride == 2 || r.mv_stride == 4) &&
+                  u64(r.mv0) + u64(r.count) * r.mv_stride <= mvs.size(),
+              "H.264: skipped-macroblock run outside the picture's pools");
+    MbRec m = r.rec;
+    for (u32 i = 0; i < r.count; ++i) {
+      m.mv = r.mv0 + i * r.mv_stride;
+      recs[r.mb0 + i] = m;
+      std::memcpy(pool + m.mv, r.mv, r.mv_stride * sizeof(i16));
+    }
+  }
+  runs_expanded = true;
+}
+
 void store_skip_mb(Picture& pic, int mb, MbRec& m, const MbState& s) {
   m.coef = u32(pic.coefs.size());
   m.luma_coded = 0;
   m.chroma_coded = 0;
   m.wp = 0;
   m.res = kNoRes;
-  store_motion(pic, m, s);
+  const u32 u = mb_motion_uniformity(m, s);
+  auto check = [&] {
+    for (int k = 0; k < 4; ++k) {
+      const int r0 = m.ref[k], r1 = m.ref1[k];
+      VEP_CHECK((r0 != 0xFF || r1 != 0xFF) && (r0 == 0xFF || r0 < pic.dpb_slots) && (r1 == 0xFF || r1 < pic.dpb_slots) &&
+                    (r1 == 0xFF || (m.flags & kMbL1)),
+                "skipped macroblock reference slot outside the DPB");
+    }
+    VEP_CHECK(m.qp <= 51 + pic.qp_bias && m.qpc <= 51 + pic.qpc_bias && m.qpc2 <= 51 + pic.qpc_bias,
+              "macroblock QP out of range");
+  };
+  if ((u & 1) && skip_runs_enabled() && (!pic.colb || (pic.colb->col->corners && pic.colb->uids))) {
+    const u32 stride = (m.flags & kMbL1) ? 4 : 2;
+    m.flags |= kMbMv16;
+    i16 mv[4] = {s.mv[0][0][0], s.mv[0][0][1], 0, 0};
+    if (stride == 4) mv[2] = s.mv[1][0][0], mv[3] = s.mv[1][0][1];
+    Picture::OpenRun& o = pic.open_run;
+    if (o.open) {
+      m.mv = o.r.rec.mv;
+      if (u32(mb) == o.r.mb0 + o.r.count && mb < o.row_end && std::memcmp(&m, &o.r.rec, sizeof m) == 0 &&
+          std::memcmp(mv, o.r.mv, sizeof mv) == 0 && std::memcmp(s.ref, o.ref, sizeof o.ref) == 0) {
+        ++o.r.count;
+        pic.mvs.extend(stride);
+        ++pic.inter_mbs;
+        return;
+      }
+      pic.flush_run();
+    }
+    check();
+    m.mv = u32(pic.mvs.size());
+    pic.mvs.extend(stride);
+    ++pic.inter_mbs;
+    if (!(m.dbk & 1)) pic.deblock = true;
+    o.open = true;
+    o.row_end = (mb / pic.wmbs + 1) * pic.wmbs;
+    o.r.mb0 = u32(mb);
+    o.r.count = 1;
+    o.r.mv0 = m.mv;
+    o.r.mv_stride = stride;
+    o.r.rec = m;
+    std::memcpy(o.r.mv, mv, sizeof mv);
+    std::memcpy(o.ref, s.ref, sizeof o.ref);
+    if (pic.colb) {
+      ColMotion::Blk col[4];
+      pic.colb->corner_entries(s, col);
+      static_assert(sizeof col == sizeof o.col, "four colocated entries");
+      std::memcpy(o.col, col, sizeof col);
+    }
+    return;
+  }
+  pic.flush_run();
+  store_motion(pic, m, s, u);
   ++pic.inter_mbs;
   if (!(m.dbk & 1)) pic.deblock = true;
-  for (int k = 0; k < 4; ++k) {
-    const int r0 = m.ref[k], r1 = m.ref1[k];
-    VEP_CHECK((r0 != 0xFF || r1 != 0xFF) && (r0 == 0xFF || r0 < pic.dpb_slots) && (r1 == 0xFF || r1 < pic.dpb_slots) &&
-                  (r1 == 0xFF || (m.flags & kMbL1)),
-              "skipped macroblock reference slot outside the DPB");
-  }
-  VEP_CHECK(m.qp <= 51 + pic.qp_bias && m.qpc <= 51 + pic.qpc_bias && m.qpc2 <= 51 + pic.qpc_bias,
-            "macroblock QP out of range");
+  check();
   store_rec(&pic.mbs[size_t(mb)], m);
   if (pic.colb) pic.colb->store(mb, s);
 }
 
 void store_mb(Picture& pic, int mb, MbRec m, const MbState& s, const MbResidual* res, const u8* pcm,
               const WpEntry* wp) {
+  pic.flush_run();
   m.coef = u32(pic.coefs.size());
   m.luma_coded = 0;
   m.chroma_coded = 0;
@@ -2150,7 +2269,7 @@
   m.wp = 0;
   m.flags &= u8(~(kMbMv8x8 | kMbMv16));
   if (m.kind == kSkip || m.kind == kInter) {
-    store_motion(pic, m, s);
+    store_motion(pic, m, s, mb_motion_uniformity(m, s));
     if (wp && (m.flags & kMbWp)) {
       m.wp = u32(pic.wps.size());
       pic.wps.insert(pic.wps.end(), wp, wp + 4);
@@ -2492,11 +2611,13 @@
 }
 
 void cpu_reconstruct_mb(const Picture& pic, int mb, std::vector<HostSurface>& slots) {
+  pic.records();
   if (slots[size_t(pic.target)].wide()) reconstruct_mb_t<u16>(pic, mb, slots);
   else reconstruct_mb_t<u8>(pic, mb, slots);
 }
 
 void cpu_deblock(const Picture& pic, HostSurface& T) {
+  pic.records();
   if (T.wide()) deblock_t<u16>(pic, T);
   else deblock_t<u8>(pic, T);
 }
@@ -2516,6 +2637,7 @@
   HostSurface& T = slots[size_t(pic.target)];
   VEP_CHECK(T.coded_w == pic.wmbs * 16 && T.coded_h == pic.hmbs * 16 && T.bd == pic.bd && T.cf == pic.cf,
             "surface size mismatch");
+  pic.records();
   for (int mb = 0; mb < pic.nmbs(); ++mb) cpu_reconstruct_mb(pic, mb, slots);
   if (pic.deblock) cpu_deblock(pic, T);
 }
diff --git a/csrc/vep/avc.h b/csrc/vep/avc.h
--- a/csrc/vep/avc.h
+++ b/csrc/vep/avc.h
@@ -52,9 +52,28 @@
   AuMeta au;
   std::vector<OutFrame> outputs;
   ColBuild* colb = nullptr;
+  hostmem::pinned_vector<SkipRun> runs;
+  int run_mbs = 0;
+  mutable bool runs_expanded = false;
+  void expand_runs() const;
+  const MbRec* records() const {
+    VEP_CHECK(runs.empty() || runs_expanded, "H.264: picture records read before expand_runs()");
+    return mbs.data();
+  }
+  struct OpenRun {
+    bool open = false;
+    int row_end = 0;
+    SkipRun r;
+    i8 ref[2][4];
+    u64 col[6];
+  } open_run;
+  void flush_run();
 
   int nmbs() const { return wmbs * hmbs; }
 };
+
+bool skip_runs_enabled();
+void set_skip_runs(int mode);
 using PicturePtr = std::shared_ptr<const Picture>;
 
 void validate(const Picture& p);
@@ -148,6 +167,7 @@
   void mb_neighbour_refs(int mb, int list, int ref[3]) const;
   void direct_spatial_pred(int mb, int list, int& ref, int mv[2]) const;
   void direct_spatial_both(int ref[2], int mv[2][2]) const;
+  bool skip_neighbours_match(const i8 ref[2], const u32 mvw[2]) const;
 
  private:
   struct Nb {
@@ -337,6 +357,24 @@
   }
 }
 
+inline bool MbNeighbours::skip_neighbours_match(const i8 ref[2], const u32 mvw[2]) const {
+  const int cm = c_ >= 0 ? c_ : d_;
+  if (a_ < 0 || a_ != cur_ - 1 || b_ < 0 || cm < 0) return false;
+  const MbState& sb = st_[size_t(b_) & mask_];
+  const MbState& sc = st_[size_t(cm) & mask_];
+  if (is_intra(sb.kind) || is_intra(sc.kind)) return false;
+  const int cblk = c_ >= 0 ? 12 : 15, cb8 = c_ >= 0 ? 2 : 3;
+  for (int l = 0; l < 2; ++l) {
+    if (sb.ref[l][2] != ref[l] || sc.ref[l][cb8] != ref[l]) return false;
+    if (ref[l] < 0) continue;
+    u32 vb, vc;
+    std::memcpy(&vb, sb.mv[l][12], 4);
+    std::memcpy(&vc, sc.mv[l][cblk], 4);
+    if (vb != mvw[l] || vc != mvw[l]) return false;
+  }
+  return true;
+}
+
 struct ColMotion {
   struct Blk {
     i16 mv[2];
@@ -362,6 +400,8 @@
   }
   void store(int mb, const MbState& st);
   void none(int mb);
+  void corner_entries(const MbState& st, ColMotion::Blk out[4]) const;
+  void fill(int mb0, int count, const void* entries);
 };
 
 struct RefPic {
@@ -464,6 +504,9 @@
   Decoder();
   ~Decoder();
   u64 parallel_slices_run() const { return parallel_slices_run_; }
+  void set_parallel_slices(bool on) { parallel_slices_ = on; }
+  bool keep_col = false;
+  std::shared_ptr<const ColMotion> last_col;
   u64 mmco_ops[7] = {0, 0, 0, 0, 0, 0, 0};
   u64 list_mods = 0, long_term_marked = 0;
   u64 redundant_slices_skipped = 0;
diff --git a/csrc/vep/avc_mb.cpp b/csrc/vep/avc_mb.cpp
--- a/csrc/vep/avc_mb.cpp
+++ b/csrc/vep/avc_mb.cpp
@@ -132,7 +132,6 @@
   bool read_skip_flag(int mb, bool v = false) {
     MbState& s = nb_.at(mb);
     if constexpr (kWrite) s = MbState{};
-    else clear_but_mv(s);
     s.slice = u16(env_.slice);
     nb_.begin(mb);
     auto cond = [&](int m) { return m >= 0 && !nb_.at(m).skip ? 1 : 0; };
@@ -140,12 +139,41 @@
     return bins->mb_skip(type_ == h264::kB, inc, v) != 0;
   }
 
+  bool continue_run(int mb, MbState& s) {
+    Picture::OpenRun& o = pic_.open_run;
+    if (!o.open || o.r.mb0 + o.r.count != u32(mb) || mb >= o.row_end) return false;
+    if (type_ != h264::kP && !fast_direct_) return false;
+    const i8 ref[2] = {o.ref[0][0], o.ref[1][0]};
+    u32 mvw[2];
+    std::memcpy(mvw, o.r.mv, sizeof mvw);
+    if (type_ != h264::kP && ((ref[0] == 0 && mvw[0]) || (ref[1] == 0 && mvw[1]))) return false;
+    if (!nb_.skip_neighbours_match(ref, mvw)) return false;
+    s = nb_.at(mb - 1);
+    nz8_ = 0;
+    pic_.mvs.extend(o.r.mv_stride);
+    ++o.r.count;
+    ++pic_.inter_mbs;
+    return true;
+  }
+
   void skip_mb(int mb, bool fresh) {
     MbState& s = nb_.at(mb);
-    if (fresh) {
-      s = MbState{};
+    prev_qpd_nz = 0;
+    if constexpr (kWrite) {
+      if (fresh) {
+        s = MbState{};
+        s.slice = u16(env_.slice);
+        nb_.begin(mb);
+      }
+    } else {
+      if (fresh) {
+        s.slice = u16(env_.slice);
+        nb_.begin(mb);
+      }
+      if (continue_run(mb, s)) return;
+      if (fresh) s = MbState{};
+      else clear_but_mv(s);
       s.slice = u16(env_.slice);
-      nb_.begin(mb);
     }
     s.kind = kSkip;
     s.skip = 1;
@@ -180,7 +208,8 @@
       s.slice = u16(env_.slice);
       nb_.begin(mb);
     } else if constexpr (!kWrite) {
-      std::memset(static_cast<void*>(s.mv), 0, sizeof s.mv);
+      s = MbState{};
+      s.slice = u16(env_.slice);
     }
     int mbt = read_mb_type(mb, kWrite ? want->mb_type : 0);
     int itype = -1;
@@ -808,6 +837,14 @@
       const bool use = ref[l] >= 0 && !zero;
       pv[l] = use ? (u32(u16(mvp[l][0])) | u32(u16(mvp[l][1])) << 16) : 0u;
       std::memset(s.ref[l], ref[l], 4);
+    }
+    if (!((ref[0] == 0 && pv[0]) || (ref[1] == 0 && pv[1]))) {
+      for (int l = 0; l < 2; ++l) {
+        u32 row[4] = {pv[l], pv[l], pv[l], pv[l]};
+        u8* mv = reinterpret_cast<u8*>(&s.mv[l][0][0]);
+        for (int y = 0; y < 4; ++y) std::memcpy(mv + 16 * y, row, 16);
+      }
+      return;
     }
     const ColMotion::Blk* cb = &dcol_->b[size_t(mb) * 4];
     u32 v8[2][4];
diff --git a/csrc/vep/avc_recon.h b/csrc/vep/avc_recon.h
--- a/csrc/vep/avc_recon.h
+++ b/csrc/vep/avc_recon.h
@@ -56,6 +56,15 @@
 };
 static_assert(sizeof(MbRec) == 56, "MbRec layout");
 constexpr u32 kNoRes = 0xFFFFFFFFu;
+
+struct SkipRun {
+  u32 mb0, count;
+  u32 mv0;
+  u32 mv_stride;
+  MbRec rec;
+  i16 mv[4];
+};
+static_assert(sizeof(SkipRun) == 80 && sizeof(SkipRun) % 8 == 0, "SkipRun layout");
 
 VEP_HD int mv_per_list(u8 flags) { return (flags & kMbMv16) ? 2 : ((flags & kMbMv8x8) ? 8 : 32); }
 VEP_HD int byte_at(const u8* a, int i) {
@@ -899,7 +908,7 @@
   if (chroma) {
     if (bs < 4) {
       const int tc = tc0 + 1;
-      const int d = clip3(-tc, tc, (((q0 - p0) << 2) + (p1 - q1) + 4) >> 3);
+      const int d = clip3(-tc, tc, ((q0 - p0) * 4 + (p1 - q1) + 4) >> 3);
       p[0] = clip1(p0 + d, bd);
       q[0] = clip1(q0 - d, bd);
     } else {
@@ -912,7 +921,7 @@
   const int ap = iabs(p2 - p0), aq = iabs(q2 - q0);
   if (bs < 4) {
     const int tc = tc0 + (ap < beta) + (aq < beta);
-    const int d = clip3(-tc, tc, (((q0 - p0) << 2) + (p1 - q1) + 4) >> 3);
+    const int d = clip3(-tc, tc, ((q0 - p0) * 4 + (p1 - q1) + 4) >> 3);
     p[0] = clip1(p0 + d, bd);
     q[0] = clip1(q0 - d, bd);
     if (ap < beta) p[1] = p1 + clip3(-tc0, tc0, (p2 + ((p0 + q0 + 1) >> 1) - (p1 << 1)) >> 1);
@@ -944,7 +953,7 @@
   const bool lp = !chroma && iabs(p2 - p0) < beta, lq = !chroma && iabs(q2 - q0) < beta;
   if (bs < 4) {
     const int tc = chroma ? tc0 + 1 : tc0 + int(lp) + int(lq);
-    const int dl = clip3(-tc, tc, (((q0 - p0) << 2) + (p1 - q1) + 4) >> 3);
+    const int dl = clip3(-tc, tc, ((q0 - p0) * 4 + (p1 - q1) + 4) >> 3);
     p[0] = clip1(p0 + dl, bd);
     q[0] = clip1(q0 - dl, bd);
     if (lp) p[1] = p1 + clip3(-tc0, tc0, (p2 + ((p0 + q0 + 1) >> 1) - (p1 << 1)) >> 1);
diff --git a/csrc/vep/gpu.h b/csrc/vep/gpu.h
--- a/csrc/vep/gpu.h
+++ b/csrc/vep/gpu.h
@@ -7,6 +7,10 @@
 #include <mutex>
 
 #include "common.h"
+
+namespace vep::avc {
+struct SkipRun;
+}
 
 namespace vep::gpu {
 
@@ -159,6 +163,9 @@
   i32 intra_mbs;
   i32 deblock;
   VEP_DEV u64* xg;
+  const VEP_DEV void* runs;
+  u32 nruns;
+  u32 pad_;
 };
 constexpr int kAvcProfSlots = 20;
 constexpr int kAvcResSamples = 512;
@@ -178,6 +185,8 @@
 }
 constexpr int kAvcMaxRows = 512;
 constexpr int kAvcMaxCols = 512;
+void launch_avc_expand_runs(const AvcDesc* d_descs, int n, int max_runs, hipStream_t s);
+void check_skip_runs(const avc::SkipRun* runs, size_t n, size_t nmbs, size_t nmv);
 void launch_avc_inter(const AvcDesc* d_descs, int n, int total_mbs, hipStream_t s);
 void launch_avc_intra(const AvcDesc* d_descs, int n, int max_hmbs, hipStream_t s);
 void launch_avc_bs(const AvcDesc* d_descs, int n, int total_mbs, hipStream_t s);
diff --git a/csrc/vep/gpu_avc.hip b/csrc/vep/gpu_avc.hip
--- a/csrc/vep/gpu_avc.hip
+++ b/csrc/vep/gpu_avc.hip
@@ -199,6 +199,29 @@
     if ((m.chroma_coded >> kb) & 1) o += avc::idct4x4_at(D + 256 + 16 * kb, cy & 3, cx & 3);
     tuv[size_t(my * CH + cy) * pitch + (mx * 8 + cx) * 2 + cc] = P(avc::clip1(o, bd));
   }
+}
+
+static_assert(sizeof(MbRec) == 7 * sizeof(u64) && offsetof(MbRec, mv) == 4 * sizeof(u64) &&
+                  offsetof(avc::SkipRun, rec) == 2 * sizeof(u64) && offsetof(avc::SkipRun, mv) == 9 * sizeof(u64),
+              "avc_expand_runs_kernel word layout");
+__global__ __launch_bounds__(256) void avc_expand_runs_kernel(const AvcDesc* __restrict__ descs) {
+  const AvcDesc& d = descs[blockIdx.y];
+  const u32 run = blockIdx.x * 4u + (threadIdx.x >> 6), lane = threadIdx.x & 63u;
+  if (run >= d.nruns) return;
+  const VEP_GLOBAL u64* r = (const VEP_GLOBAL u64*)(d.runs) + size_t(run) * (sizeof(avc::SkipRun) / sizeof(u64));
+  const u64 w0 = r[0], w1 = r[1], mvw = r[9];
+  const u32 mb0 = u32(w0), count = u32(w0 >> 32), mv0 = u32(w1), stride = u32(w1 >> 32);
+  VEP_GLOBAL u64* recs = (VEP_GLOBAL u64*)(d.mbs) + size_t(mb0) * 7u;
+  const u32 nw = count * 7u;
+  for (u32 w = lane; w < nw; w += 64u) {
+    const u32 i = w / 7u, f = w - i * 7u;
+    u64 v = r[2u + f];
+    if (f == 4u) v = (v & 0xFFFFFFFF00000000ull) | u64(mv0 + i * stride);
+    recs[w] = v;
+  }
+  VEP_GLOBAL u32* mvs = (VEP_GLOBAL u32*)(d.mvs) + (mv0 >> 1);
+  const u32 per = stride >> 1, nv = count * per;
+  for (u32 k = lane; k < nv; k += 64u) mvs[k] = (k & (per - 1u)) ? u32(mvw >> 32) : u32(mvw);
 }
 
 __global__ __launch_bounds__(256) void avc_inter_kernel(const AvcDesc* __restrict__ descs, int n,
@@ -1258,6 +1281,30 @@
   VEP_HIP(hipGetLastError());
 }
 
+void check_skip_runs(const avc::SkipRun* runs, size_t n, size_t nmbs, size_t nmv) {
+  VEP_CHECK(n == 0 || runs, "skip runs: null descriptors");
+  u64 mb_end = 0, mv_end = 0;
+  for (size_t k = 0; k < n; ++k) {
+    const avc::SkipRun& r = runs[k];
+    VEP_CHECK(r.count >= 1 && r.mb0 >= mb_end && u64(r.mb0) + r.count <= nmbs,
+              "skip runs: macroblocks outside the record array or not ascending");
+    const bool l1 = (r.rec.flags & avc::kMbL1) != 0;
+    VEP_CHECK(r.mv_stride == (l1 ? 4u : 2u) && (r.rec.flags & avc::kMbMv16) && r.rec.mv == r.mv0 && r.mv0 % 2 == 0,
+              "skip runs: motion stride, granularity or offset differs from the template record");
+    VEP_CHECK(r.mv0 >= mv_end && u64(r.mv0) + u64(r.count) * r.mv_stride <= nmv,
+              "skip runs: motion entries outside the pool or not ascending");
+    mb_end = u64(r.mb0) + r.count;
+    mv_end = u64(r.mv0) + u64(r.count) * r.mv_stride;
+  }
+}
+
+void launch_avc_expand_runs(const AvcDesc* d_descs, int n, int max_runs, hipStream_t s) {
+  if (n <= 0 || max_runs <= 0) return;
+  hipLaunchKernelGGL(avc_expand_runs_kernel, dim3(unsigned((max_runs + 3) / 4), unsigned(n)), dim3(256), 0, s,
+                     d_descs);
+  VEP_HIP(hipGetLastError());
+}
+
 void launch_avc_inter(const AvcDesc* d_descs, int n, int total_mbs, hipStream_t s) {
   if (n <= 0 || total_mbs <= 0) return;
   hipLaunchKernelGGL(avc_inter_kernel, dim3(unsigned((total_mbs + 3) / 4)), dim3(256), 0, s, d_descs, n,
diff --git a/csrc/vep/runtime.cpp b/csrc/vep/runtime.cpp
--- a/csrc/vep/runtime.cpp
+++ b/csrc/vep/runtime.cpp
@@ -1328,7 +1328,29 @@
   struct AvcPic {
     const avc::Picture* p;
     int job;
-    size_t off_mbs, off_coef, off_mv, off_wp, off_dbk, off_res, off_xg;
+    size_t off_mbs, off_coef, off_mv, off_wp, off_runs, off_dbk, off_res, off_xg;
+    std::vector<u8> skip_mbs;
+  };
+  auto run_chunks = [](const avc::Picture& p) {
+    std::vector<u8> skip;
+    if (p.runs.empty()) return skip;
+    const size_t bytes = p.mbs.size() * sizeof(avc::MbRec);
+    skip.assign((bytes + gpu::kGatherChunk - 1) / gpu::kGatherChunk, 0);
+    size_t lo = 0, hi = 0;
+    auto mark = [&] {
+      const size_t c0 = (lo * sizeof(avc::MbRec) + gpu::kGatherChunk - 1) / gpu::kGatherChunk;
+      const size_t end = hi * sizeof(avc::MbRec);
+      for (size_t c = c0; c < skip.size() && std::min(bytes, (c + 1) * size_t(gpu::kGatherChunk)) <= end; ++c) skip[c] = 1;
+    };
+    for (const avc::SkipRun& r : p.runs) {
+      if (r.mb0 != hi) {
+        mark();
+        lo = r.mb0;
+      }
+      hi = size_t(r.mb0) + r.count;
+    }
+    mark();
+    return skip;
   };
   std::vector<AvcPic> apics;
   int rounds = 0;
@@ -1345,7 +1367,7 @@
       VEP_CHECK(p.wmbs * 16 == jobs[size_t(i)].pic.coded_width &&
                     p.hmbs * 16 * (p.structure ? 2 : 1) == jobs[size_t(i)].pic.coded_height,
                 "picture size differs from the camera's surfaces");
-      AvcPic a{&p, i, 0, 0, 0, 0, 0, 0, 0};
+      AvcPic a{&p, i, 0, 0, 0, 0, 0, 0, 0, 0, {}};
       auto put = [&](const void* src, size_t bytes) {
         const size_t o = need;
         need += al(bytes);
@@ -1353,9 +1375,14 @@
         return o;
       };
       a.off_mbs = put(p.mbs.data(), p.mbs.size() * sizeof(avc::MbRec));
+      if (pinned(p.mbs.data(), p.mbs.size() * sizeof(avc::MbRec))) {
+        a.skip_mbs = run_chunks(p);
+        for (u8 s : a.skip_mbs) nchunks -= s;
+      }
       a.off_coef = put(p.coefs.data(), p.coefs.size() * sizeof(i16));
       a.off_mv = put(p.mvs.data(), p.mvs.size() * sizeof(i16));
       a.off_wp = put(p.wps.data(), p.wps.size() * sizeof(avc::WpEntry));
+      a.off_runs = put(p.runs.data(), p.runs.size() * sizeof(avc::SkipRun));
       round_pics[size_t(r)].push_back(int(apics.size()));
       apics.push_back(a);
     }
@@ -1507,21 +1534,25 @@
   auto* gc = reinterpret_cast<gpu::GatherChunk*>(st.h + off_gather);
   size_t ng = 0;
   for (const AvcPic& a : apics) {
-    auto add = [&](const void* src, size_t len, size_t off) {
+    auto add = [&](const void* src, size_t len, size_t off, const std::vector<u8>* skip = nullptr) {
       if (pinned(src, len)) {
         const u8* dv = hostmem::device_address(static_cast<const u8*>(src), len);
-        for (size_t o = 0; o < len; o += gpu::kGatherChunk)
-          gc[ng++] = {dv + o, st.d + off + o, u32(std::min<size_t>(gpu::kGatherChunk, len - o)), 0};
-        records_gathered_ += u64(len);
+        for (size_t o = 0; o < len; o += gpu::kGatherChunk) {
+          const size_t n = std::min<size_t>(gpu::kGatherChunk, len - o);
+          if (skip && !skip->empty() && (*skip)[o / gpu::kGatherChunk]) continue;
+          gc[ng++] = {dv + o, st.d + off + o, u32(n), 0};
+          records_gathered_ += u64(n);
+        }
         return;
       }
       for (size_t o = 0; o < len; o += kPackChunk)
         tasks.push_back({static_cast<const u8*>(src) + o, st.h + off + o, std::min(kPackChunk, len - o)});
     };
-    add(a.p->mbs.data(), a.p->mbs.size() * sizeof(avc::MbRec), a.off_mbs);
+    add(a.p->mbs.data(), a.p->mbs.size() * sizeof(avc::MbRec), a.off_mbs, &a.skip_mbs);
     add(a.p->coefs.data(), a.p->coefs.size() * sizeof(i16), a.off_coef);
     add(a.p->mvs.data(), a.p->mvs.size() * sizeof(i16), a.off_mv);
     add(a.p->wps.data(), a.p->wps.size() * sizeof(avc::WpEntry), a.off_wp);
+    add(a.p->runs.data(), a.p->runs.size() * sizeof(avc::SkipRun), a.off_runs);
   }
   for (const HevcPic& a : hpics) {
     auto add = [&](const void* src, size_t len, size_t off) {
@@ -1760,6 +1791,10 @@
       g.nres = u32(a.p->intra_res);
       g.intra_mbs = a.p->intra_mbs;
       g.deblock = a.p->deblock ? 1 : 0;
+      gpu::check_skip_runs(a.p->runs.data(), a.p->runs.size(), a.p->mbs.size(), a.p->mvs.size());
+      g.runs = st.d + a.off_runs;
+      g.nruns = u32(a.p->runs.size());
+      g.pad_ = 0;
       VEP_CHECK(c->surface.bd == a.p->bd && c->surface.cf == a.p->cf,
                 "H.264: picture bit depth / chroma format differs from the camera's surfaces");
       mbs += a.p->nmbs();
@@ -1873,8 +1908,9 @@
     int mbs = 0;
     bool intra = false, dbk = false, narrow = false;
     int variants = 0;
-    int max_h = 0;
+    int max_h = 0, max_runs = 0;
     for (int k : round_pics[size_t(r)]) {
+      max_runs = std::max(max_runs, int(apics[size_t(k)].p->runs.size()));
       mbs += apics[size_t(k)].p->nmbs();
       max_h = std::max(max_h, apics[size_t(k)].p->hmbs);
       intra |= apics[size_t(k)].p->intra_mbs > 0;
@@ -1883,6 +1919,7 @@
       if (ap.bd > 8 || ap.cf == 2) variants |= ap.cf != 2 ? 1 : (ap.bd > 8 ? 4 : 2);
       else narrow = true;
     }
+    gpu::launch_avc_expand_runs(ad, np, max_runs, cs);
     gpu::launch_avc_inter(ad, np, mbs, cs);
     if (intra && narrow) gpu::launch_avc_intra(ad, np, max_h, cs);
     if (dbk) {
@@ -2011,6 +2048,7 @@
       };
       for (size_t k = 0; k < jobs[i].avc.size(); ++k) {
         const auto& pic = jobs[i].avc[k];
+        pic->expand_runs();
         if (!pic->structure) {
           avc::cpu_reconstruct(*pic, c.surface.host);
           convert_history(k);
```
